# lukecq1231/nats

Measured on NVIDIA H100. Metric: decoder tokens/sec (dim=1000, src=400, |V|=30k) @1/2/4/8 H100 vs Theano CPU, higher is better.
Workload: dtype f32

## Files before the change

### include/nats_b200.h

```cpp
#ifndef NATS_B200_H
#define NATS_B200_H

#include <stdint.h>
#include <stddef.h>

#ifdef __cplusplus
extern "C" {
#endif

#pragma GCC visibility push(default)

#define NATS_NUM_PARAMS 43
#define NATS_GRAD_TAIL 32

typedef struct nats_ctx nats_ctx_t;

typedef struct {
    int32_t n_words;
    int32_t dim_word;
    int32_t dim;
    int32_t dim_att;
} nats_dims_t;

typedef struct {
    char name[32];
    int64_t offset;
    int32_t rows, cols, ld;
    int32_t ndim;
} nats_param_view_t;

const char* nats_last_error(void);
int nats_version(void);

int nats_ctx_create(int device, nats_ctx_t** out);
int nats_ctx_destroy(nats_ctx_t* ctx);

int nats_param_layout(const nats_dims_t* dims, nats_param_view_t* views, int64_t* total_floats);

int64_t nats_train_workspace_bytes(const nats_dims_t* dims, int Tx, int Ty, int B);

int nats_train_fwd(nats_ctx_t* ctx, void* stream, const nats_dims_t* dims, const float* params,
                   const int64_t* x, const float* x_mask, const int64_t* y, const float* y_mask,
                   int Tx, int Ty, int B, void* ws, int64_t ws_bytes, float* cost);

int nats_train_bwd(nats_ctx_t* ctx, void* stream, const nats_dims_t* dims, const float* params,
                   const int64_t* x, const float* x_mask, const int64_t* y, const float* y_mask,
                   int Tx, int Ty, int B, void* ws, int64_t ws_bytes, float scale, float* grads);

int64_t nats_grad_split(const nats_dims_t* dims);
int nats_train_bwd_begin(nats_ctx_t* ctx, void* stream, const nats_dims_t* dims, const float* params,
                         const int64_t* x, const float* x_mask, const int64_t* y, const float* y_mask,
                         int Tx, int Ty, int B, void* ws, int64_t ws_bytes, float scale, float* grads);
int nats_train_bwd_finish(nats_ctx_t* ctx, void* stream, const nats_dims_t* dims, const float* params,
                          const int64_t* x, const float* x_mask, const int64_t* y, const float* y_mask,
                          int Tx, int Ty, int B, void* ws, int64_t ws_bytes, float scale, float* grads);

int nats_encoder_fwd(nats_ctx_t* ctx, void* stream, const nats_dims_t* dims, const float* params,
                     const int64_t* x, const float* x_mask , int Tx, int Ty, int B,
                     void* ws, int64_t ws_bytes);
int nats_decoder_scan_fwd(nats_ctx_t* ctx, void* stream, const nats_dims_t* dims, const float* params,
                          const int64_t* y, const float* x_mask, const float* y_mask, int Tx, int Ty, int B,
                          void* ws, int64_t ws_bytes);
int nats_readout_nll_fwd(nats_ctx_t* ctx, void* stream, const nats_dims_t* dims, const float* params,
                         const int64_t* y, const float* y_mask, int Tx, int Ty, int B,
                         void* ws, int64_t ws_bytes, float* cost);
int nats_readout_nll_bwd(nats_ctx_t* ctx, void* stream, const nats_dims_t* dims, const float* params,
                         const int64_t* y, const float* y_mask, int Tx, int Ty, int B,
                         void* ws, int64_t ws_bytes, float scale, float* grads);
int nats_decoder_scan_bwd(nats_ctx_t* ctx, void* stream, const nats_dims_t* dims, const float* params,
                          const int64_t* y, const float* x_mask, const float* y_mask, int Tx, int Ty, int B,
                          void* ws, int64_t ws_bytes, float* grads);
int nats_encoder_bwd(nats_ctx_t* ctx, void* stream, const nats_dims_t* dims, const float* params,
                     const int64_t* x, const float* x_mask, const int64_t* y, int Tx, int Ty, int B,
                     void* ws, int64_t ws_bytes, float* grads);

const float* nats_train_ws_view(const nats_dims_t* dims, int Tx, int Ty, int B, void* ws, const char* name);

int64_t nats_sampler_workspace_bytes(const nats_dims_t* dims, int Tx, int n);

int nats_sampler_init(nats_ctx_t* ctx, void* stream, const nats_dims_t* dims, const float* params,
                      const int64_t* x, const float* x_mask, int Tx, int n, void* ws, int64_t ws_bytes,
                      float* init_state, float* ctx_out, float* pctx_out);

int nats_sampler_next(nats_ctx_t* ctx, void* stream, const nats_dims_t* dims, const float* params,
                      const int64_t* y, const float* ctx_in, int64_t ctx_tstride, int64_t ctx_bstride,
                      const float* pctx_in, int64_t pctx_tstride, int64_t pctx_bstride,
                      const float* state, const float* acc_ctx, const float* acc_alpha, int Tx, int n,
                      uint64_t rng_seed, uint64_t rng_step, void* ws, int64_t ws_bytes,
                      float* probs, int64_t* sample, float* state_out, float* alphaT, float* ctxs,
                      float* acc_ctx_out, float* acc_alpha_out);

int nats_grad_clip(nats_ctx_t* ctx, void* stream, int64_t n, const float* params, float* grads,
                   float decay_c, float clip_c, float* stats );

int nats_adadelta_grad_shared(nats_ctx_t* ctx, void* stream, int64_t n, const float* zg, float* rg2, float rho);
int nats_adadelta_update(nats_ctx_t* ctx, void* stream, int64_t n, float* params, const float* zg,
                         float* ru2, const float* rg2, float rho, float eps);
int nats_adam_update(nats_ctx_t* ctx, void* stream, int64_t n, float* params, const float* g,
                     float* m, float* v, int64_t step);
int nats_rmsprop_grad_shared(nats_ctx_t* ctx, void* stream, int64_t n, const float* zg, float* rg, float* rg2);
int nats_rmsprop_update(nats_ctx_t* ctx, void* stream, int64_t n, float* params, const float* zg,
                        float* ud, const float* rg, const float* rg2);

int nats_beam_distraction_scores(nats_ctx_t* ctx, void* stream,
                                 const float* hist_alpha, const float* hist_ctx, const float* hist_state,
                                 int len_cap, int hist_len, int live_k, int Tx, int C, int D,
                                 const float* cur_alpha, const float* cur_ctx, const float* cur_state,
                                 float kl_factor, float ctx_factor, float state_factor,
                                 float* scratch, float* out);

int nats_beam_topk(nats_ctx_t* ctx, void* stream, const float* probs , int n, int n_words, int k,
                   int mask_unk, float* out_p , int32_t* out_idx );

int nats_beam_reorder_append(nats_ctx_t* ctx, void* stream, const float* src, float* dst, const float* cur,
                             const int32_t* parent, int n_new, int len_cap, int hist_len, int dim);

int nats_beam_select(nats_ctx_t* ctx, void* stream, const float* top_p, const int32_t* top_i, const float* pen,
                     int k, int maxlen, int step, int32_t* counters, float* scores, int32_t* tokens, int32_t* parents,
                     int64_t* next_w, int32_t* out_tokens, int32_t* out_len, float* out_score, int32_t* fin_parent,
                     int32_t* host_counters);
int nats_beam_advance(nats_ctx_t* ctx, void* stream, const int32_t* parents, const int32_t* fin_parent,
                      const int32_t* counters, int k, int len_cap, int step, int Tx, int C, int D,
                      const float* state_o, float* state_n, const float* acc_ctx_o, float* acc_ctx_n,
                      const float* acc_alpha_o, float* acc_alpha_n,
                      const float* cur_alpha, const float* cur_ctx, const float* cur_state,
                      const float* hist_alpha_src, float* hist_alpha_dst, const float* hist_ctx_src, float* hist_ctx_dst,
                      const float* hist_state_src, float* hist_state_dst, float* out_alpha);

typedef struct nats_beam_step {
    const float* params;
    const int64_t* next_w;
    const float* ctx; const float* pctx;
    int32_t Tx, k, maxlen, use_unk;
    void* ws; int64_t ws_bytes;
    const float* state_in; const float* acc_ctx_in; const float* acc_alpha_in;
    float* probs; float* state_out; float* alphaT; float* ctxs; float* acc_ctx_out; float* acc_alpha_out;
    float kl_factor, ctx_factor, state_factor;
    const float* hist_alpha_in; const float* hist_ctx_in; const float* hist_state_in;
    float* scratch; float* pen;
    float* top_p; int32_t* top_i;
    int32_t* counters; float* scores; int32_t* tokens; int32_t* parents; int32_t* fin_parent;
    int32_t* out_tokens; int32_t* out_len; float* out_score; float* out_alpha; int32_t* host_counters;
    float* state_next; float* acc_ctx_next; float* acc_alpha_next;
    float* hist_alpha_out; float* hist_ctx_out; float* hist_state_out;
} nats_beam_step_t;
int nats_beam_step(nats_ctx_t* ctx, void* stream, const nats_dims_t* dims, const nats_beam_step_t* a, int step);

typedef struct nats_beam_step_many {
    nats_beam_step_t beam;
    int32_t n_src;
    const int32_t* src_len;
} nats_beam_step_many_t;
int nats_beam_step_many(nats_ctx_t* ctx, void* stream, const nats_dims_t* dims, const nats_beam_step_many_t* a, int step);

int nats_debug_gemm(nats_ctx_t* ctx, void* stream, int path, int transA, int transB, int M, int N, int K,
                    const float* A, int lda, const float* B, int ldb, float* C, int ldc, const float* bias,
                    int accumulate, int splitk, int batch, int64_t strideA, int64_t strideB, int64_t strideC);

int nats_profile_enable(nats_ctx_t* ctx, int on);
int nats_profile_num_classes(void);
const char* nats_profile_class_name(int cls);
int nats_profile_read(nats_ctx_t* ctx, int n_classes, double* ms, double* flops, double* bytes, int64_t* launches);

#pragma GCC visibility pop

#ifdef __cplusplus
}
#endif
#endif
```

### nats_b200/_lib.py

```python
import ctypes
import os
from ctypes import (POINTER, Structure, c_char, c_char_p, c_double, c_float, c_int, c_int32, c_int64, c_uint64,
                    c_void_p)

_HERE = os.path.dirname(os.path.abspath(__file__))
LIB_PATH = os.path.join(_HERE, 'libnats_b200.so')
HEADER_PATH = os.path.join(os.path.dirname(_HERE), 'include', 'nats_b200.h')

NUM_PARAMS = 43
GRAD_TAIL = 32


class Dims(Structure):
    _fields_ = [('n_words', c_int32), ('dim_word', c_int32), ('dim', c_int32), ('dim_att', c_int32)]


class ParamView(Structure):
    _fields_ = [('name', c_char * 32), ('offset', c_int64), ('rows', c_int32), ('cols', c_int32),
                ('ld', c_int32), ('ndim', c_int32)]


_P = c_void_p


class BeamStep(Structure):
    _fields_ = ([('params', _P), ('next_w', _P), ('ctx', _P), ('pctx', _P),
                 ('Tx', c_int32), ('k', c_int32), ('maxlen', c_int32), ('use_unk', c_int32),
                 ('ws', _P), ('ws_bytes', c_int64)] +
                [(n, _P) for n in ('state_in', 'acc_ctx_in', 'acc_alpha_in', 'probs', 'state_out', 'alphaT', 'ctxs',
                                   'acc_ctx_out', 'acc_alpha_out')] +
                [('kl_factor', c_float), ('ctx_factor', c_float), ('state_factor', c_float)] +
                [(n, _P) for n in ('hist_alpha_in', 'hist_ctx_in', 'hist_state_in', 'scratch', 'pen', 'top_p', 'top_i',
                                   'counters', 'scores', 'tokens', 'parents', 'fin_parent', 'out_tokens', 'out_len',
                                   'out_score', 'out_alpha', 'host_counters', 'state_next', 'acc_ctx_next',
                                   'acc_alpha_next', 'hist_alpha_out', 'hist_ctx_out', 'hist_state_out')])


class BeamStepMany(Structure):
    _fields_ = [('beam', BeamStep), ('n_src', c_int32), ('src_len', _P)]

SIGNATURES = {
    'nats_last_error': (c_char_p, []),
    'nats_version': (c_int, []),
    'nats_ctx_create': (c_int, [c_int, POINTER(c_void_p)]),
    'nats_ctx_destroy': (c_int, [c_void_p]),
    'nats_param_layout': (c_int, [POINTER(Dims), POINTER(ParamView), POINTER(c_int64)]),
    'nats_train_workspace_bytes': (c_int64, [POINTER(Dims), c_int, c_int, c_int]),
    'nats_train_fwd': (c_int, [c_void_p, _P, POINTER(Dims), _P, _P, _P, _P, _P, c_int, c_int, c_int, _P, c_int64, _P]),
    'nats_train_bwd': (c_int, [c_void_p, _P, POINTER(Dims), _P, _P, _P, _P, _P, c_int, c_int, c_int, _P, c_int64,
                               c_float, _P]),
    'nats_grad_split': (c_int64, [POINTER(Dims)]),
    'nats_train_bwd_begin': (c_int, [c_void_p, _P, POINTER(Dims), _P, _P, _P, _P, _P, c_int, c_int, c_int, _P, c_int64,
                                     c_float, _P]),
    'nats_train_bwd_finish': (c_int, [c_void_p, _P, POINTER(Dims), _P, _P, _P, _P, _P, c_int, c_int, c_int, _P, c_int64,
                                      c_float, _P]),
    'nats_encoder_fwd': (c_int, [c_void_p, _P, POINTER(Dims), _P, _P, _P, c_int, c_int, c_int, _P, c_int64]),
    'nats_decoder_scan_fwd': (c_int, [c_void_p, _P, POINTER(Dims), _P, _P, _P, _P, c_int, c_int, c_int, _P, c_int64]),
    'nats_readout_nll_fwd': (c_int, [c_void_p, _P, POINTER(Dims), _P, _P, _P, c_int, c_int, c_int, _P, c_int64, _P]),
    'nats_readout_nll_bwd': (c_int, [c_void_p, _P, POINTER(Dims), _P, _P, _P, c_int, c_int, c_int, _P, c_int64,
                                     c_float, _P]),
    'nats_decoder_scan_bwd': (c_int, [c_void_p, _P, POINTER(Dims), _P, _P, _P, _P, c_int, c_int, c_int, _P, c_int64,
                                      _P]),
    'nats_encoder_bwd': (c_int, [c_void_p, _P, POINTER(Dims), _P, _P, _P, _P, c_int, c_int, c_int, _P, c_int64, _P]),
    'nats_train_ws_view': (c_void_p, [POINTER(Dims), c_int, c_int, c_int, _P, c_char_p]),
    'nats_sampler_workspace_bytes': (c_int64, [POINTER(Dims), c_int, c_int]),
    'nats_sampler_init': (c_int, [c_void_p, _P, POINTER(Dims), _P, _P, _P, c_int, c_int, _P, c_int64, _P, _P, _P]),
    'nats_sampler_next': (c_int, [c_void_p, _P, POINTER(Dims), _P, _P, _P, c_int64, c_int64, _P, c_int64, c_int64,
                                  _P, _P, _P, c_int, c_int, c_uint64, c_uint64, _P, c_int64,
                                  _P, _P, _P, _P, _P, _P, _P]),
    'nats_grad_clip': (c_int, [c_void_p, _P, c_int64, _P, _P, c_float, c_float, _P]),
    'nats_adadelta_grad_shared': (c_int, [c_void_p, _P, c_int64, _P, _P, c_float]),
    'nats_adadelta_update': (c_int, [c_void_p, _P, c_int64, _P, _P, _P, _P, c_float, c_float]),
    'nats_adam_update': (c_int, [c_void_p, _P, c_int64, _P, _P, _P, _P, c_int64]),
    'nats_rmsprop_grad_shared': (c_int, [c_void_p, _P, c_int64, _P, _P, _P]),
    'nats_rmsprop_update': (c_int, [c_void_p, _P, c_int64, _P, _P, _P, _P, _P]),
    'nats_beam_distraction_scores': (c_int, [c_void_p, _P, _P, _P, _P, c_int, c_int, c_int, c_int, c_int, c_int,
                                             _P, _P, _P, c_float, c_float, c_float, _P, _P]),
    'nats_beam_topk': (c_int, [c_void_p, _P, _P, c_int, c_int, c_int, c_int, _P, _P]),
    'nats_beam_reorder_append': (c_int, [c_void_p, _P, _P, _P, _P, _P, c_int, c_int, c_int, c_int]),
    'nats_beam_select': (c_int, [c_void_p, _P, _P, _P, _P, c_int, c_int, c_int, _P, _P, _P, _P, _P, _P, _P, _P, _P, _P]),
    'nats_beam_advance': (c_int, [c_void_p, _P] + [_P] * 3 + [c_int] * 6 + [_P] * 16),
    'nats_beam_step': (c_int, [c_void_p, _P, POINTER(Dims), POINTER(BeamStep), c_int]),
    'nats_beam_step_many': (c_int, [c_void_p, _P, POINTER(Dims), POINTER(BeamStepMany), c_int]),
    'nats_debug_gemm': (c_int, [c_void_p, _P, c_int, c_int, c_int, c_int, c_int, c_int, _P, c_int, _P, c_int, _P, c_int,
                                _P, c_int, c_int, c_int, c_int64, c_int64, c_int64]),
    'nats_profile_enable': (c_int, [c_void_p, c_int]),
    'nats_profile_num_classes': (c_int, []),
    'nats_profile_class_name': (c_char_p, [c_int]),
    'nats_profile_read': (c_int, [c_void_p, c_int, POINTER(c_double), POINTER(c_double), POINTER(c_double),
                                  POINTER(c_int64)]),
}

_lib = None


class NatsB200Error(RuntimeError):
    pass


def load():
    global _lib
    if _lib is not None:
        return _lib
    if not os.path.exists(LIB_PATH):
        raise NatsB200Error('%s not found: build it with `python nats_b200/csrc/build.py` '
                            '(or __graft_entry__.build()); nats_b200 has no CPU fallback' % LIB_PATH)
    lib = ctypes.CDLL(LIB_PATH)
    for name, (res, args) in SIGNATURES.items():
        fn = getattr(lib, name)
        fn.restype = res
        fn.argtypes = args
    _lib = lib
    return lib


def check(rc, what=''):
    if rc != 0:
        msg = load().nats_last_error()
        raise NatsB200Error('%s failed (rc=%d): %s' % (what or 'libnats_b200 call', rc,
                                                      msg.decode() if msg else '?'))


def param_layout(n_words, dim_word, dim, dim_att):
    lib = load()
    d = Dims(n_words, dim_word, dim, dim_att)
    views = (ParamView * NUM_PARAMS)()
    total = c_int64(0)
    check(lib.nats_param_layout(ctypes.byref(d), views, ctypes.byref(total)), 'nats_param_layout')
    out = [(v.name.decode(), v.offset, v.rows, v.cols, v.ld, v.ndim) for v in views]
    return out, total.value
```

### nats_b200/csrc/api.cu

```cuda
#include <stdarg.h>
#include <stdlib.h>

#include <vector>

#include "model.cuh"

namespace nats {
static thread_local char g_err[1024] = "";
void set_error(const char* fmt, ...) {
    va_list ap;
    va_start(ap, fmt);
    vsnprintf(g_err, sizeof(g_err), fmt, ap);
    va_end(ap);
}
}

namespace nats {
namespace {
struct ProfRec { int cls; double flops, bytes; };
struct ProfState {
    bool on = false;
    std::vector<cudaEvent_t> ev;
    std::vector<ProfRec> recs;
};
ProfState g_prof;
const char* kNames[K_COUNT] = {
    "gemm_big_nn", "gemm_big_nt", "gemm_big_tn", "gemm_big_tt", "gemm_mid_nn", "gemm_mid_nt", "gemm_mid_tn",
    "gemm_mid_tt", "gemm_smallm_nn", "gemm_smallm_nt", "gemm_smallm_tn", "gemm_smallm_tt", "gru_gates_fwd",
    "gru_gates_bwd", "att_scores", "att_context", "att_bwd_ctx", "att_bwd_dalpha", "att_bwd_softmax", "nll_rows",
    "dlogits", "softmax_sample", "colsum", "reduce_splits", "embedding", "elementwise", "optimizer", "beam",
    "memset", "tc_gemm_3xtf32", "tc_gemm_3xtf32_skinny", "enc_tc_fwd", "enc_tc_bwd"};
}
const char* kclass_name(int cls) { return (cls >= 0 && cls < K_COUNT) ? kNames[cls] : "?"; }
bool prof_enabled() { return g_prof.on; }
void prof_begin(cudaStream_t st, int cls, double flops, double bytes) {
    const size_t i = g_prof.recs.size();
    while (g_prof.ev.size() < 2 * (i + 1)) {
        cudaEvent_t e;
        if (cudaEventCreate(&e) != cudaSuccess) { g_prof.on = false; return; }
        g_prof.ev.push_back(e);
    }
    g_prof.recs.push_back(ProfRec{cls, flops, bytes});
    cudaEventRecord(g_prof.ev[2 * i], st);
}
void prof_end(cudaStream_t st) {
    if (g_prof.recs.empty()) return;
    cudaEventRecord(g_prof.ev[2 * (g_prof.recs.size() - 1) + 1], st);
}
}

namespace nats {
static int g_pdl = 1;
int pdl_enabled() { return g_pdl; }
void pdl_set(int on) { g_pdl = on; }
}

using namespace nats;

namespace {

int check_dims(const nats_dims_t* d) {
    NATS_REQUIRE(d != nullptr, "dims");
    NATS_REQUIRE(d->n_words >= 2 && d->dim_word >= 1 && d->dim >= 1 && d->dim_att >= 1, "dims must be positive");
    NATS_REQUIRE(d->dim_att <= 256, "dim_att <= 256");
    return 0;
}

struct ViewDef { const char* name; int64_t off; int rows, cols, ld, ndim; };

}

extern "C" {

const char* nats_last_error(void) { return g_err; }
int nats_version(void) { return 101; }

int nats_ctx_create(int device, nats_ctx_t** out) {
    NATS_REQUIRE(out != nullptr, "out");
    NATS_CUDA_OK(cudaSetDevice(device));
    cudaDeviceProp prop;
    NATS_CUDA_OK(cudaGetDeviceProperties(&prop, device));
    if (prop.major != 9 || prop.minor != 0) {
        set_error("libnats_b200 is built for sm_90a only; device %d is sm_%d%d", device, prop.major, prop.minor);
        return 3;
    }
    nats_ctx* c = new nats_ctx;
    c->device = device;
    c->num_sms = prop.multiProcessorCount;
    c->max_smem_optin = (int)prop.sharedMemPerBlockOptin;
    c->dev_scratch = nullptr;
    NATS_CUDA_OK(cudaMalloc(&c->dev_scratch, kCtxScratchFloats * sizeof(float)));
    int r = attention_setup(c);
    if (r == 0) r = narrow_proj_setup(c);
    if (r == 0) r = tc_gemm_setup();
    if (r == 0) r = tma_gemm_setup();
    if (r == 0) r = enc_tc_setup(c);
    enc_tc_enable(getenv("NATS_ENC_TC") ? atoi(getenv("NATS_ENC_TC")) : 1);
    attention_set_cc_keep(getenv("NATS_CC_KEEP") ? atoi(getenv("NATS_CC_KEEP")) : 0);
    tma_gemm_set_ts(getenv("NATS_TS") ? atoi(getenv("NATS_TS")) : 1);
    if (getenv("NATS_TRACE_GATES")) gates_trace(atoi(getenv("NATS_TRACE_GATES")));
    pdl_set(getenv("NATS_PDL") ? atoi(getenv("NATS_PDL")) : 1);
    gemm_set_tensor_cores(getenv("NATS_TC") ? atoi(getenv("NATS_TC")) : 2);
    if (r != 0) { cudaFree(c->dev_scratch); delete c; return r; }
    *out = c;
    return 0;
}

int nats_ctx_destroy(nats_ctx_t* ctx) {
    if (!ctx) return 0;
    if (ctx->dev_scratch) cudaFree(ctx->dev_scratch);
    delete ctx;
    return 0;
}

int nats_param_layout(const nats_dims_t* dims, nats_param_view_t* views, int64_t* total_floats) {
    NATS_TRY(check_dims(dims));
    const ParamOff o = param_offsets(*dims);
    const int V = dims->n_words, W = dims->dim_word, D = dims->dim, A = dims->dim_att, C = 2 * D, D3 = 3 * D;
    const ViewDef defs[NATS_NUM_PARAMS] = {
        {"Wemb", o.Wemb, V, W, W, 2},
        {"encoder_W", o.enc[0].Wcat, W, 2 * D, D3, 2},
        {"encoder_b", o.enc[0].bcat, 1, 2 * D, D3, 1},
        {"encoder_U", o.enc[0].Ucat, D, 2 * D, D3, 2},
        {"encoder_Wx", o.enc[0].Wcat + 2 * D, W, D, D3, 2},
        {"encoder_bx", o.enc[0].bcat + 2 * D, 1, D, D3, 1},
        {"encoder_Ux", o.enc[0].Ucat + 2 * D, D, D, D3, 2},
        {"encoder_r_W", o.enc[1].Wcat, W, 2 * D, D3, 2},
        {"encoder_r_b", o.enc[1].bcat, 1, 2 * D, D3, 1},
        {"encoder_r_U", o.enc[1].Ucat, D, 2 * D, D3, 2},
        {"encoder_r_Wx", o.enc[1].Wcat + 2 * D, W, D, D3, 2},
        {"encoder_r_bx", o.enc[1].bcat + 2 * D, 1, D, D3, 1},
        {"encoder_r_Ux", o.enc[1].Ucat + 2 * D, D, D, D3, 2},
        {"ff_state_W", o.ff_state_W, C, D, D, 2},
        {"ff_state_b", o.ff_state_b, 1, D, D, 1},
        {"decoder_W", o.dec.Wcat, W, 2 * D, D3, 2},
        {"decoder_U", o.dec.Ucat, D, 2 * D, D3, 2},
        {"decoder_b", o.dec.bcat, 1, 2 * D, D3, 1},
        {"decoder_Wx", o.dec.Wcat + 2 * D, W, D, D3, 2},
        {"decoder_Ux", o.dec.Ucat + 2 * D, D, D, D3, 2},
        {"decoder_bx", o.dec.bcat + 2 * D, 1, D, D3, 1},
        {"decoder_U_1", o.U1cat, D, 2 * D, D3, 2},
        {"decoder_W_1", o.W1cat, C, 2 * D, D3, 2},
        {"decoder_b_1", o.b1cat, 1, 2 * D, D3, 1},
        {"decoder_Wx_1", o.W1cat + 2 * D, C, D, D3, 2},
        {"decoder_Ux_1", o.U1cat + 2 * D, D, D, D3, 2},
        {"decoder_bx_1", o.b1cat + 2 * D, 1, D, D3, 1},
        {"decoder_W_att", o.W_att, D, A, A, 2},
        {"decoder_Wc_att", o.Wc_att, C, A, A, 2},
        {"decoder_b_att", o.b_att, 1, A, A, 1},
        {"decoder_U_att", o.U_att, A, 1, 1, 2},
        {"decoder_c_att", o.c_att, 1, 1, 1, 1},
        {"decoder_W_con", o.W_con, C, 1, 1, 2},
        {"decoder_U_con", o.U_con, C, 1, 1, 2},
        {"decoder_D_wei", o.D_wei, 1, A, A, 2},
        {"ff_logit_lstm_W", o.lstm_W, D, W, W, 2},
        {"ff_logit_lstm_b", o.lstm_b, 1, W, W, 1},
        {"ff_logit_prev_W", o.prev_W, W, W, W, 2},
        {"ff_logit_prev_b", o.prev_b, 1, W, W, 1},
        {"ff_logit_ctx_W", o.ctxr_W, C, W, W, 2},
        {"ff_logit_ctx_b", o.ctxr_b, 1, W, W, 1},
        {"ff_logit_W", o.logit_W, W, V, V, 2},
        {"ff_logit_b", o.logit_b, 1, V, V, 1},
    };
    if (views) {
        for (int i = 0; i < NATS_NUM_PARAMS; ++i) {
            memset(&views[i], 0, sizeof(views[i]));
            strncpy(views[i].name, defs[i].name, sizeof(views[i].name) - 1);
            views[i].offset = defs[i].off;
            views[i].rows = defs[i].rows; views[i].cols = defs[i].cols; views[i].ld = defs[i].ld;
            views[i].ndim = defs[i].ndim;
        }
    }
    if (total_floats) *total_floats = o.total;
    return 0;
}

int nats_debug_gemm(nats_ctx_t* ctx, void* stream, int path, int transA, int transB, int M, int N, int K,
                    const float* A, int lda, const float* B, int ldb, float* C, int ldc, const float* bias,
                    int accumulate, int splitk, int batch, int64_t strideA, int64_t strideB, int64_t strideC) {
    NATS_REQUIRE(ctx && A && B && C, "null argument");
    GemmProblem p = gemm_problem(A, lda, B, ldb, C, ldc, M, N, K);
    p.bias = bias; p.accumulate = accumulate; p.batch = batch < 1 ? 1 : batch;
    p.strideA = strideA; p.strideB = strideB; p.strideC = strideC;
    if (splitk > 1) gemm_set_split(p, splitk, (long long)M * ldc);
    cudaStream_t st = reinterpret_cast<cudaStream_t>(stream);
    if (path == 1) return tc_gemm_launch(st, &p, 1, transA != 0, transB != 0);
    if (path == 2 || path == 3) {
        NATS_REQUIRE(tma_gemm_eligible(&p, 1), "operands not TMA-compatible (alignment)");
        const int keep_ts = tma_gemm_get_ts();
        tma_gemm_set_ts(path == 3 ? 1 : 0);
        const int r = tma_gemm_launch(st, &p, 1, transA != 0, transB != 0);
        tma_gemm_set_ts(keep_ts);
        return r;
    }
    const int keep = gemm_get_tensor_cores();
    gemm_set_tensor_cores(0);
    const int r = gemm_launch(st, &p, 1, transA != 0, transB != 0, GEMM_CFG_AUTO);
    gemm_set_tensor_cores(keep);
    return r;
}

int nats_profile_enable(nats_ctx_t* ctx, int on) {
    (void)ctx;
    g_prof.recs.clear();
    g_prof.on = on != 0;
    return 0;
}
int nats_profile_num_classes(void) { return K_COUNT; }
const char* nats_profile_class_name(int cls) { return kclass_name(cls); }
int nats_profile_read(nats_ctx_t* ctx, int n_classes, double* ms, double* flops, double* bytes, int64_t* launches) {
    (void)ctx;
    NATS_REQUIRE(n_classes >= K_COUNT && ms && flops && bytes && launches, "profile_read buffers");
    NATS_CUDA_OK(cudaDeviceSynchronize());
    for (int i = 0; i < n_classes; ++i) { ms[i] = 0; flops[i] = 0; bytes[i] = 0; launches[i] = 0; }
    for (size_t i = 0; i < g_prof.recs.size(); ++i) {
        float t = 0.f;
        if (cudaEventElapsedTime(&t, g_prof.ev[2 * i], g_prof.ev[2 * i + 1]) != cudaSuccess) continue;
        const ProfRec& r = g_prof.recs[i];
        ms[r.cls] += t; flops[r.cls] += r.flops; bytes[r.cls] += r.bytes; launches[r.cls] += 1;
    }
    g_prof.recs.clear();
    return 0;
}

int64_t nats_train_workspace_bytes(const nats_dims_t* dims, int Tx, int Ty, int B) {
    if (check_dims(dims) != 0 || Tx < 1 || Ty < 1 || B < 1) return -1;
    return carve_train(*dims, Tx, Ty, B, nullptr).bytes;
}

#define NATS_TRAIN_PROLOGUE()                                                                      \
    NATS_REQUIRE(ctx != nullptr, "ctx");                                                           \
    NATS_TRY(check_dims(dims));                                                                    \
    NATS_REQUIRE(Tx >= 1 && Ty >= 1 && B >= 1, "shape");                                           \
    NATS_REQUIRE(ws != nullptr, "workspace");                                                      \
    const TrainWS w = carve_train(*dims, Tx, Ty, B, ws);                                           \
    NATS_REQUIRE(ws_bytes >= w.bytes, "workspace too small (see nats_train_workspace_bytes)");     \
    cudaStream_t st = reinterpret_cast<cudaStream_t>(stream)

int nats_encoder_fwd(nats_ctx_t* ctx, void* stream, const nats_dims_t* dims, const float* params, const int64_t* x,
                     const float* x_mask, int Tx, int Ty, int B, void* ws, int64_t ws_bytes) {
    NATS_TRAIN_PROLOGUE();
    return train_encoder_fwd(ctx, st, *dims, params, x, x_mask, Tx, B, w);
}

int nats_decoder_scan_fwd(nats_ctx_t* ctx, void* stream, const nats_dims_t* dims, const float* params,
                          const int64_t* y, const float* x_mask, const float* y_mask, int Tx, int Ty, int B, void* ws,
                          int64_t ws_bytes) {
    NATS_TRAIN_PROLOGUE();
    return train_decoder_fwd(ctx, st, *dims, params, y, x_mask, y_mask, Tx, Ty, B, w);
}

int nats_readout_nll_fwd(nats_ctx_t* ctx, void* stream, const nats_dims_t* dims, const float* params,
                         const int64_t* y, const float* y_mask, int Tx, int Ty, int B, void* ws, int64_t ws_bytes,
                         float* cost) {
    NATS_TRAIN_PROLOGUE();
    return train_readout_fwd(ctx, st, *dims, params, y, y_mask, Ty, B, w, cost);
}

int nats_readout_nll_bwd(nats_ctx_t* ctx, void* stream, const nats_dims_t* dims, const float* params,
                         const int64_t* y, const float* y_mask, int Tx, int Ty, int B, void* ws, int64_t ws_bytes,
                         float scale, float* grads) {
    NATS_TRAIN_PROLOGUE();
    return train_readout_bwd(ctx, st, *dims, params, y, y_mask, Ty, B, w, scale, grads);
}

int nats_decoder_scan_bwd(nats_ctx_t* ctx, void* stream, const nats_dims_t* dims, const float* params,
                          const int64_t* y, const float* x_mask, const float* y_mask, int Tx, int Ty, int B, void* ws,
                          int64_t ws_bytes, float* grads) {
    NATS_TRAIN_PROLOGUE();
    return train_decoder_bwd(ctx, st, *dims, params, y, x_mask, y_mask, Tx, Ty, B, w, grads);
}

int nats_encoder_bwd(nats_ctx_t* ctx, void* stream, const nats_dims_t* dims, const float* params, const int64_t* x,
                     const float* x_mask, const int64_t* y, int Tx, int Ty, int B, void* ws, int64_t ws_bytes,
                     float* grads) {
    NATS_TRAIN_PROLOGUE();
    return train_encoder_bwd(ctx, st, *dims, params, x, x_mask, y, Tx, Ty, B, w, grads);
}

int nats_train_fwd(nats_ctx_t* ctx, void* stream, const nats_dims_t* dims, const float* params, const int64_t* x,
                   const float* x_mask, const int64_t* y, const float* y_mask, int Tx, int Ty, int B, void* ws,
                   int64_t ws_bytes, float* cost) {
    NATS_TRAIN_PROLOGUE();
    NATS_REQUIRE(x && x_mask && y && y_mask && cost && params, "null argument");
    NATS_TRY(train_encoder_fwd(ctx, st, *dims, params, x, x_mask, Tx, B, w));
    NATS_TRY(train_decoder_fwd(ctx, st, *dims, params, y, x_mask, y_mask, Tx, Ty, B, w));
    NATS_TRY(train_readout_fwd(ctx, st, *dims, params, y, y_mask, Ty, B, w, cost));
    return 0;
}

int64_t nats_grad_split(const nats_dims_t* dims) {
    if (check_dims(dims) != 0) return -1;
    return param_offsets(*dims).ff_state_W;
}

int nats_train_bwd_begin(nats_ctx_t* ctx, void* stream, const nats_dims_t* dims, const float* params, const int64_t* x,
                         const float* x_mask, const int64_t* y, const float* y_mask, int Tx, int Ty, int B, void* ws,
                         int64_t ws_bytes, float scale, float* grads) {
    NATS_TRAIN_PROLOGUE();
    NATS_REQUIRE(x && x_mask && y && y_mask && grads && params, "null argument");
    const ParamOff o = param_offsets(*dims);
    NATS_CUDA_OK(memset_async(st, grads, 0, (size_t)(o.total + NATS_GRAD_TAIL) * sizeof(float)));
    NATS_TRY(cost_reduce(st, w.rowcost, Ty, B, nullptr, scale, grads + o.total));
    NATS_TRY(train_readout_bwd(ctx, st, *dims, params, y, y_mask, Ty, B, w, scale, grads));
    NATS_TRY(train_decoder_bwd(ctx, st, *dims, params, y, x_mask, y_mask, Tx, Ty, B, w, grads));
    return 0;
}

int nats_train_bwd_finish(nats_ctx_t* ctx, void* stream, const nats_dims_t* dims, const float* params, const int64_t* x,
                          const float* x_mask, const int64_t* y, const float* y_mask, int Tx, int Ty, int B, void* ws,
                          int64_t ws_bytes, float scale, float* grads) {
    (void)scale; (void)y_mask;
    NATS_TRAIN_PROLOGUE();
    NATS_REQUIRE(x && x_mask && y && grads && params, "null argument");
    return train_encoder_bwd(ctx, st, *dims, params, x, x_mask, y, Tx, Ty, B, w, grads);
}

int nats_train_bwd(nats_ctx_t* ctx, void* stream, const nats_dims_t* dims, const float* params, const int64_t* x,
                   const float* x_mask, const int64_t* y, const float* y_mask, int Tx, int Ty, int B, void* ws,
                   int64_t ws_bytes, float scale, float* grads) {
    NATS_TRY(nats_train_bwd_begin(ctx, stream, dims, params, x, x_mask, y, y_mask, Tx, Ty, B, ws, ws_bytes, scale, grads));
    return nats_train_bwd_finish(ctx, stream, dims, params, x, x_mask, y, y_mask, Tx, Ty, B, ws, ws_bytes, scale, grads);
}

const float* nats_train_ws_view(const nats_dims_t* dims, int Tx, int Ty, int B, void* ws, const char* name) {
    if (check_dims(dims) != 0 || !ws || !name) return nullptr;
    const TrainWS w = carve_train(*dims, Tx, Ty, B, ws);
    if (!strcmp(name, "ctx")) return w.cc;
    if (!strcmp(name, "init_state")) return w.init_state;
    if (!strcmp(name, "dec_h")) return w.d_h2;
    if (!strcmp(name, "dec_ctx")) return w.d_ctx;
    if (!strcmp(name, "dec_alpha")) return w.d_alpha;
    if (!strcmp(name, "pctx")) return w.pctx;
    if (!strcmp(name, "logits")) return w.logits;
    return nullptr;
}

int64_t nats_sampler_workspace_bytes(const nats_dims_t* dims, int Tx, int n) {
    if (check_dims(dims) != 0 || Tx < 1 || n < 1) return -1;
    return carve_sampler(*dims, Tx, n, nullptr).bytes;
}

int nats_sampler_init(nats_ctx_t* ctx, void* stream, const nats_dims_t* dims, const float* params, const int64_t* x,
                      const float* x_mask, int Tx, int n, void* ws, int64_t ws_bytes, float* init_state, float* ctx_out,
                      float* pctx_out) {
    NATS_REQUIRE(ctx && ws && params && x && init_state && ctx_out, "null argument");
    NATS_TRY(check_dims(dims));
    NATS_REQUIRE(Tx >= 1 && n >= 1, "shape");
    const SamplerWS w = carve_sampler(*dims, Tx, n, ws);
    NATS_REQUIRE(ws_bytes >= w.bytes, "workspace too small (see nats_sampler_workspace_bytes)");
    cudaStream_t st = reinterpret_cast<cudaStream_t>(stream);
    EncBufs e;
    memset(&e, 0, sizeof(e));
    e.emb_x = w.emb_x;
    e.xproj[0] = w.xproj[0]; e.xproj[1] = w.xproj[1];
    e.cc = ctx_out; e.ctxsum = w.ctxsum; e.xlen = w.xlen; e.xinv = w.xinv; e.ctx_mean = w.ctx_mean;
    e.init_state = init_state; e.part_a = w.part_a;
    e.gemm_scratch = w.gemm_scratch; e.gemm_scratch_floats = w.gemm_scratch_floats;
    e.enc_scratch = w.enc_scratch; e.enc_scratch_floats = w.enc_scratch_floats;
    e.enc_counters = w.enc_counters; e.enc_counter_ints = w.enc_counter_ints;
    NATS_TRY(encoder_forward(ctx, st, *dims, params, x, x_mask, Tx, n, e));
    if (pctx_out) {
        const ParamOff o = param_offsets(*dims);
        const int A = dims->dim_att, C = 2 * dims->dim;
        GemmProblem p = gemm_problem(ctx_out, C, params + o.Wc_att, A, pctx_out, A, Tx * n, A, C);
        p.bias = params + o.b_att;
        NATS_TRY(gemm_auto(ctx, st, p, false, false, w.gemm_scratch, w.gemm_scratch_floats));
    }
    return 0;
}

}

namespace {

int sampler_next(nats_ctx_t* ctx, void* stream, const nats_dims_t* dims, const float* params, const int64_t* y,
                 const float* ctx_in, int64_t ctx_tstride, int64_t ctx_bstride, const float* pctx_in,
                 int64_t pctx_tstride, int64_t pctx_bstride, int rows_per_src, const int32_t* src_len, const float* state,
                 const float* acc_ctx, const float* acc_alpha, int Tx, int n, uint64_t rng_seed, uint64_t rng_step, void* ws,
                 int64_t ws_bytes, float* probs, int64_t* sample, float* state_out, float* alphaT, float* ctxs,
                 float* acc_ctx_out, float* acc_alpha_out) {
    NATS_REQUIRE(ctx && ws && params && y && ctx_in && state && acc_ctx && acc_alpha, "null argument");
    NATS_REQUIRE(probs && state_out && alphaT && ctxs && acc_ctx_out && acc_alpha_out, "null output");
    NATS_TRY(check_dims(dims));
    NATS_REQUIRE(Tx >= 1 && n >= 1, "shape");
    const SamplerWS w = carve_sampler(*dims, Tx, n, ws);
    NATS_REQUIRE(ws_bytes >= w.bytes, "workspace too small (see nats_sampler_workspace_bytes)");
    cudaStream_t st = reinterpret_cast<cudaStream_t>(stream);
    const ParamOff o = param_offsets(*dims);
    const int W = dims->dim_word, D = dims->dim, A = dims->dim_att, V = dims->n_words, C = 2 * D, D3 = 3 * D;

    NATS_TRY(gather_rows(st, params + o.Wemb, y, n, W, V, 0, w.emb_y));
    {
        GemmProblem p = gemm_problem(w.emb_y, W, params + o.dec.Wcat, D3, w.xproj_y, D3, n, D3, W);
        p.bias = params + o.dec.bcat;
        NATS_TRY(gemm_auto(ctx, st, p, false, false, w.gemm_scratch, w.gemm_scratch_floats));
    }
    const float* pctx = pctx_in;
    long long pts = pctx_tstride, pbs = pctx_bstride;
    if (!pctx) {
        GemmProblem p;
        if (ctx_bstride == 0) {
            p = gemm_problem(ctx_in, (int)ctx_tstride, params + o.Wc_att, A, w.pctx, A, Tx, A, C);
            pts = A; pbs = 0;
        } else {
            NATS_REQUIRE(ctx_bstride == C && ctx_tstride == (int64_t)n * C, "pctx recompute needs a dense [Tx,n,C] context");
            p = gemm_problem(ctx_in, C, params + o.Wc_att, A, w.pctx, A, Tx * n, A, C);
            pts = (long long)n * A; pbs = A;
        }
        p.bias = params + o.b_att;
        NATS_TRY(gemm_auto(ctx, st, p, false, false, w.gemm_scratch, w.gemm_scratch_floats));
        pctx = w.pctx;
    }
    DecStep s;
    memset(&s, 0, sizeof(s));
    s.n = n; s.Tx = Tx;
    s.h_prev = state; s.xproj = w.xproj_y;
    s.ymask = nullptr; s.xmask = nullptr;
    s.rows_per_src = rows_per_src; s.src_len = src_len;
    s.pctx = pctx; s.pctx_ts = pts; s.pctx_bs = pbs;
    s.cc = ctx_in; s.cc_ts = ctx_tstride; s.cc_bs = ctx_bstride;
    s.acc_alpha_in = acc_alpha; s.acc_ctx_in = acc_ctx;
    s.h1 = w.h1; s.ps_save = w.ps; s.escore = w.escore;
    s.alpha_out = alphaT; s.acc_alpha_out = acc_alpha_out; s.craw_out = w.craw; s.ctx_out = ctxs;
    s.acc_ctx_out = acc_ctx_out; s.h2 = state_out;
    s.part_a = w.part_a; s.part_b = w.part_b; s.part_c = w.part_c; s.part_d = w.part_d;
    NATS_TRY(decoder_step_forward(ctx, st, *dims, params, s));

    NarrowProj np;
    memset(&np, 0, sizeof(np));
    np.x[0] = state_out; np.ldx[0] = D; np.W[0] = params + o.lstm_W; np.ldw[0] = W; np.bias[0] = params + o.lstm_b; np.K[0] = D;
    np.x[1] = w.emb_y;   np.ldx[1] = W; np.W[1] = params + o.prev_W; np.ldw[1] = W; np.bias[1] = params + o.prev_b; np.K[1] = W;
    np.x[2] = ctxs;      np.ldx[2] = C; np.W[2] = params + o.ctxr_W; np.ldw[2] = W; np.bias[2] = params + o.ctxr_b; np.K[2] = C;
    np.n = n; np.N = W; np.out = w.L; np.ldo = W; np.act_tanh = 1;
    GemmProblem p;
    if (narrow_proj_eligible(np)) {
        NATS_TRY(narrow_proj(st, np));
    } else {
        p = gemm_problem(state_out, D, params + o.lstm_W, W, w.L, W, n, W, D);
        p.bias = params + o.lstm_b;
        NATS_TRY(gemm_auto(ctx, st, p, false, false, w.gemm_scratch, w.gemm_scratch_floats));
        p = gemm_problem(w.emb_y, W, params + o.prev_W, W, w.L, W, n, W, W);
        p.bias = params + o.prev_b; p.accumulate = 1;
        NATS_TRY(gemm_auto(ctx, st, p, false, false, w.gemm_scratch, w.gemm_scratch_floats));
        p = gemm_problem(ctxs, C, params + o.ctxr_W, W, w.L, W, n, W, C);
        p.bias = params + o.ctxr_b; p.accumulate = 1;
        NATS_TRY(gemm_auto(ctx, st, p, false, false, w.gemm_scratch, w.gemm_scratch_floats));
        NATS_TRY(tanh_inplace(st, w.L, (long long)n * W));
    }
    p = gemm_problem(w.L, W, params + o.logit_W, V, w.logits, V, n, V, W);
    p.bias = params + o.logit_b;
    NATS_TRY(gemm_auto(ctx, st, p, false, false, w.gemm_scratch, w.gemm_scratch_floats));
    NATS_TRY(softmax_sample_rows(st, w.logits, n, V, probs, sample, rng_seed, rng_step));
    return 0;
}

}

extern "C" {

int nats_sampler_next(nats_ctx_t* ctx, void* stream, const nats_dims_t* dims, const float* params, const int64_t* y,
                      const float* ctx_in, int64_t ctx_tstride, int64_t ctx_bstride, const float* pctx_in,
                      int64_t pctx_tstride, int64_t pctx_bstride, const float* state, const float* acc_ctx,
                      const float* acc_alpha, int Tx, int n, uint64_t rng_seed, uint64_t rng_step, void* ws,
                      int64_t ws_bytes, float* probs, int64_t* sample, float* state_out, float* alphaT, float* ctxs,
                      float* acc_ctx_out, float* acc_alpha_out) {
    return sampler_next(ctx, stream, dims, params, y, ctx_in, ctx_tstride, ctx_bstride, pctx_in, pctx_tstride, pctx_bstride,
                        ctx_bstride == 0 ? n : 1, nullptr, state, acc_ctx, acc_alpha, Tx, n, rng_seed, rng_step, ws, ws_bytes,
                        probs, sample, state_out, alphaT, ctxs, acc_ctx_out, acc_alpha_out);
}

int nats_grad_clip(nats_ctx_t* ctx, void* stream, int64_t n, const float* params, float* grads, float decay_c,
                   float clip_c, float* stats) {
    NATS_REQUIRE(ctx && grads && stats, "null argument");
    NATS_REQUIRE(!(decay_c > 0.f) || params, "params needed for decay");
    return grad_clip(ctx, reinterpret_cast<cudaStream_t>(stream), n, params, grads, decay_c, clip_c, stats);
}
int nats_adadelta_grad_shared(nats_ctx_t* ctx, void* stream, int64_t n, const float* zg, float* rg2, float rho) {
    (void)ctx;
    return adadelta_grad_shared(reinterpret_cast<cudaStream_t>(stream), n, zg, rg2, rho);
}
int nats_adadelta_update(nats_ctx_t* ctx, void* stream, int64_t n, float* params, const float* zg, float* ru2,
                         const float* rg2, float rho, float eps) {
    (void)ctx;
    return adadelta_update(reinterpret_cast<cudaStream_t>(stream), n, params, zg, ru2, rg2, rho, eps);
}
int nats_adam_update(nats_ctx_t* ctx, void* stream, int64_t n, float* params, const float* g, float* m, float* v,
                     int64_t step) {
    (void)ctx;
    return adam_update(reinterpret_cast<cudaStream_t>(stream), n, params, g, m, v, step);
}
int nats_rmsprop_grad_shared(nats_ctx_t* ctx, void* stream, int64_t n, const float* zg, float* rg, float* rg2) {
    (void)ctx;
    return rmsprop_grad_shared(reinterpret_cast<cudaStream_t>(stream), n, zg, rg, rg2);
}
int nats_rmsprop_update(nats_ctx_t* ctx, void* stream, int64_t n, float* params, const float* zg, float* ud,
                        const float* rg, const float* rg2) {
    (void)ctx;
    return rmsprop_update(reinterpret_cast<cudaStream_t>(stream), n, params, zg, ud, rg, rg2);
}

int nats_beam_distraction_scores(nats_ctx_t* ctx, void* stream, const float* hist_alpha, const float* hist_ctx,
                                 const float* hist_state, int len_cap, int hist_len, int live_k, int Tx, int C, int D,
                                 const float* cur_alpha, const float* cur_ctx, const float* cur_state, float kl_factor,
                                 float ctx_factor, float state_factor, float* scratch, float* out) {
    (void)ctx;
    return beam_distraction_scores(reinterpret_cast<cudaStream_t>(stream), hist_alpha, hist_ctx, hist_state, len_cap,
                                   hist_len, live_k, Tx, C, D, cur_alpha, cur_ctx, cur_state, kl_factor, ctx_factor,
                                   state_factor, nullptr, 0, scratch, out);
}
int nats_beam_topk(nats_ctx_t* ctx, void* stream, const float* probs, int n, int n_words, int k, int mask_unk,
                   float* out_p, int32_t* out_idx) {
    (void)ctx;
    return beam_topk(reinterpret_cast<cudaStream_t>(stream), probs, n, n_words, k, mask_unk, out_p, out_idx);
}

int nats_beam_reorder_append(nats_ctx_t* ctx, void* stream, const float* src, float* dst, const float* cur,
                             const int32_t* parent, int n_new, int len_cap, int hist_len, int dim) {
    (void)ctx;
    return beam_reorder_append(reinterpret_cast<cudaStream_t>(stream), src, dst, cur, parent, n_new, len_cap, hist_len,
                               dim);
}

int nats_beam_select(nats_ctx_t* ctx, void* stream, const float* top_p, const int32_t* top_i, const float* pen, int k,
                     int maxlen, int step, int32_t* counters, float* scores, int32_t* tokens, int32_t* parents,
                     int64_t* next_w, int32_t* out_tokens, int32_t* out_len, float* out_score, int32_t* fin_parent,
                     int32_t* host_counters) {
    (void)ctx;
    NATS_REQUIRE(top_p && top_i && counters && scores && tokens && parents && next_w && out_tokens && out_len && out_score &&
                     fin_parent, "null argument");
    return beam_select(reinterpret_cast<cudaStream_t>(stream), top_p, top_i, pen, 1, k, maxlen, step, counters, scores, tokens,
                       parents, reinterpret_cast<long long*>(next_w), out_tokens, out_len, out_score, fin_parent, host_counters);
}

int nats_beam_advance(nats_ctx_t* ctx, void* stream, const int32_t* parents, const int32_t* fin_parent,
                      const int32_t* counters, int k, int len_cap, int step, int Tx, int C, int D, const float* state_o,
                      float* state_n, const float* acc_ctx_o, float* acc_ctx_n, const float* acc_alpha_o, float* acc_alpha_n,
                      const float* cur_alpha, const float* cur_ctx, const float* cur_state, const float* hist_alpha_src,
                      float* hist_alpha_dst, const float* hist_ctx_src, float* hist_ctx_dst, const float* hist_state_src,
                      float* hist_state_dst, float* out_alpha) {
    (void)ctx;
    NATS_REQUIRE(parents && fin_parent && counters && state_o && state_n && acc_ctx_o && acc_ctx_n && acc_alpha_o &&
                     acc_alpha_n && cur_alpha && hist_alpha_src && hist_alpha_dst && out_alpha, "null argument");
    NATS_REQUIRE(hist_ctx_src == nullptr || (hist_ctx_dst && hist_state_src && hist_state_dst && cur_ctx && cur_state),
                 "context / state histories come together");
    return beam_advance(reinterpret_cast<cudaStream_t>(stream), parents, fin_parent, counters, 1, k, len_cap, step, Tx, C, D,
                        state_o, state_n, acc_ctx_o, acc_ctx_n, acc_alpha_o, acc_alpha_n, cur_alpha, cur_ctx, cur_state,
                        hist_alpha_src, hist_alpha_dst, hist_ctx_src, hist_ctx_dst, hist_state_src, hist_state_dst, out_alpha);
}

}

namespace {

int beam_step_group(nats_ctx_t* ctx, cudaStream_t st, const nats_dims_t* dims, const nats_beam_step_t* a, int n_src,
                    const int32_t* src_len, int step) {
    NATS_REQUIRE(ctx && dims && a, "null argument");
    NATS_REQUIRE(a->k >= 1 && a->k <= 32 && a->maxlen >= 1 && step >= 0 && step < a->maxlen, "beam step shape (1 <= k <= 32)");
    NATS_REQUIRE(n_src >= 1 && (long long)n_src * a->k <= 65535, "beam group size");
    NATS_TRY(check_dims(dims));
    const int D = dims->dim, C = 2 * D, A = dims->dim_att, V = dims->n_words, k = a->k, Tx = a->Tx, n = n_src * k;
    void* stream = reinterpret_cast<void*>(st);
    const int64_t cbs = n_src == 1 ? 0 : C, pbs = n_src == 1 ? 0 : A;
    NATS_TRY(sampler_next(ctx, stream, dims, a->params, a->next_w, a->ctx, (int64_t)n_src * C, cbs, a->pctx, (int64_t)n_src * A,
                          pbs, k, src_len, a->state_in, a->acc_ctx_in, a->acc_alpha_in, Tx, n, 0, 0, a->ws, a->ws_bytes,
                          a->probs, nullptr, a->state_out, a->alphaT, a->ctxs, a->acc_ctx_out, a->acc_alpha_out));
    const bool distract = a->kl_factor > 0.f || a->ctx_factor > 0.f || a->state_factor > 0.f;
    const bool use_pen = distract && step > 0;
    if (use_pen) {
        NATS_REQUIRE(a->hist_ctx_in && a->hist_state_in && a->scratch && a->pen, "distraction buffers");
        NATS_TRY(beam_distraction_scores(st, a->hist_alpha_in, a->hist_ctx_in, a->hist_state_in, a->maxlen, step, n, Tx, C, D,
                                         a->alphaT, a->ctxs, a->state_out, a->kl_factor, a->ctx_factor, a->state_factor,
                                         a->counters, k, a->scratch, a->pen));
    }
    NATS_REQUIRE(a->probs && a->top_p && a->top_i && a->counters && a->scores && a->tokens && a->parents && a->next_w &&
                     a->out_tokens && a->out_len && a->out_score && a->fin_parent, "null argument");
    NATS_REQUIRE(a->state_next && a->acc_ctx_next && a->acc_alpha_next && a->hist_alpha_in && a->hist_alpha_out && a->out_alpha,
                 "null argument");
    NATS_REQUIRE(!distract || (a->hist_ctx_out && a->hist_state_out), "distraction histories");
    NATS_TRY(beam_topk(st, a->probs, n, V, k, a->use_unk ? 0 : 1, a->top_p, a->top_i));
    NATS_TRY(beam_select(st, a->top_p, a->top_i, use_pen ? a->pen : nullptr, n_src, k, a->maxlen, step, a->counters, a->scores,
                         a->tokens, a->parents, reinterpret_cast<long long*>(const_cast<int64_t*>(a->next_w)), a->out_tokens,
                         a->out_len, a->out_score, a->fin_parent, a->host_counters));
    NATS_TRY(beam_advance(st, a->parents, a->fin_parent, a->counters, n_src, k, a->maxlen, step, Tx, C, D, a->state_out,
                          a->state_next, a->acc_ctx_out, a->acc_ctx_next, a->acc_alpha_out, a->acc_alpha_next, a->alphaT, a->ctxs,
                          a->state_out, a->hist_alpha_in, a->hist_alpha_out, distract ? a->hist_ctx_in : nullptr,
                          a->hist_ctx_out, a->hist_state_in, a->hist_state_out, a->out_alpha));
    return 0;
}

}

extern "C" {

int nats_beam_step(nats_ctx_t* ctx, void* stream, const nats_dims_t* dims, const nats_beam_step_t* a, int step) {
    return beam_step_group(ctx, reinterpret_cast<cudaStream_t>(stream), dims, a, 1, nullptr, step);
}

int nats_beam_step_many(nats_ctx_t* ctx, void* stream, const nats_dims_t* dims, const nats_beam_step_many_t* a, int step) {
    NATS_REQUIRE(a != nullptr, "null argument");
    NATS_REQUIRE(a->n_src >= 1, "n_src >= 1");
    NATS_REQUIRE(a->src_len != nullptr, "src_len");
    return beam_step_group(ctx, reinterpret_cast<cudaStream_t>(stream), dims, &a->beam, a->n_src, a->src_len, step);
}


}
```

### nats_b200/csrc/gemm.cuh

```cuda
#pragma once
#include "common.cuh"

namespace nats {


struct GemmProblem {
    const float* A;
    const float* B;
    float* C;
    const float* bias;
    int M, N, K;
    int lda, ldb, ldc;
    int batch;
    long long strideA, strideB, strideC;
    int splitk;
    int kchunk;
    long long strideP;
    int accumulate;
};

constexpr int kGemmMaxGroup = 4;
constexpr int kGemmMaxSplit = 32;

struct GemmGroup {
    GemmProblem p[kGemmMaxGroup];
    int zstart[kGemmMaxGroup + 1];
    int count;
};

enum GemmCfg { GEMM_CFG_AUTO = 0, GEMM_CFG_BIG = 1, GEMM_CFG_MID = 2, GEMM_CFG_SMALLM = 3 };

inline GemmProblem gemm_problem(const float* A, int lda, const float* B, int ldb, float* C, int ldc,
                                int M, int N, int K) {
    GemmProblem p;
    memset(&p, 0, sizeof(p));
    p.A = A; p.B = B; p.C = C; p.bias = nullptr;
    p.M = M; p.N = N; p.K = K; p.lda = lda; p.ldb = ldb; p.ldc = ldc;
    p.batch = 1; p.splitk = 1; p.kchunk = ((K + 15) / 16) * 16; if (p.kchunk == 0) p.kchunk = 16;
    p.accumulate = 0;
    return p;
}
inline void gemm_set_split(GemmProblem& p, int splits, long long strideP) {
    if (splits < 1) splits = 1;
    int chunk = (p.K + splits - 1) / splits;
    chunk = ((chunk + 15) / 16) * 16;
    if (chunk == 0) chunk = 16;
    p.kchunk = chunk;
    p.splitk = splits;
    p.strideP = strideP;
}

int tc_gemm_launch(cudaStream_t st, const GemmProblem* probs, int count, bool transA, bool transB);
int tc_gemm_setup();
int tma_gemm_launch(cudaStream_t st, const GemmProblem* probs, int count, bool transA, bool transB);
bool tma_gemm_eligible(const GemmProblem* probs, int count);
int tma_gemm_setup();
void gemm_set_tensor_cores(int on);
int gemm_get_tensor_cores();

int gemm_launch(cudaStream_t st, const GemmProblem* probs, int count, bool transA, bool transB, int cfg);

int gemm_step_cfg(int M);
int gemm_pick_split(const nats_ctx* ctx, int M, int N, int K, int groups = 1);

int gemm_auto(const nats_ctx* ctx, cudaStream_t st, GemmProblem p, bool transA, bool transB,
              float* scratch, long long scratch_floats);

int reduce_splits(cudaStream_t st, const float* part, int nsplit, long long strideP, int M, int N, int ldp,
                  float* out, int ldo, const float* bias, int accumulate);

}
```

### nats_b200/csrc/model_bwd.cu

```cuda
#include "model.cuh"

namespace nats {

namespace {
inline int ga(const nats_ctx* ctx, cudaStream_t st, const TrainWS& w, GemmProblem p, bool ta, bool tb) {
    return gemm_auto(ctx, st, p, ta, tb, w.gemm_scratch, w.gemm_scratch_floats);
}
}

int train_readout_bwd(const nats_ctx* ctx, cudaStream_t st, const nats_dims_t& d, const float* params,
                      const int64_t* y, const float* y_mask, int Ty, int B, const TrainWS& w, float scale,
                      float* G) {
    const ParamOff o = param_offsets(d);
    const int W = d.dim_word, D = d.dim, V = d.n_words, C = 2 * D;
    const int YB = Ty * B;
    NATS_TRY(dlogits_inplace(st, w.logits, YB, V, y, y_mask, w.lse, scale));
    NATS_TRY(ga(ctx, st, w, gemm_problem(w.L, W, w.logits, V, G + o.logit_W, V, W, V, YB), true, false));
    NATS_TRY(colsum(st, w.logits, YB, V, V, G + o.logit_b, 0, w.red_scratch));
    NATS_TRY(ga(ctx, st, w, gemm_problem(w.logits, V, params + o.logit_W, V, w.dpre, W, YB, W, V), false, true));
    NATS_TRY(dtanh(st, w.dpre, w.L, w.dpre, (long long)YB * W));
    NATS_TRY(ga(ctx, st, w, gemm_problem(w.d_h2, D, w.dpre, W, G + o.lstm_W, W, D, W, YB), true, false));
    NATS_TRY(ga(ctx, st, w, gemm_problem(w.embs, W, w.dpre, W, G + o.prev_W, W, W, W, YB), true, false));
    NATS_TRY(ga(ctx, st, w, gemm_problem(w.d_ctx, C, w.dpre, W, G + o.ctxr_W, W, C, W, YB), true, false));
    NATS_TRY(colsum3(st, w.dpre, YB, W, W, G + o.lstm_b, G + o.prev_b, G + o.ctxr_b, 0, w.red_scratch));
    NATS_TRY(ga(ctx, st, w, gemm_problem(w.dpre, W, params + o.lstm_W, W, w.dh2_ro, D, YB, D, W), false, true));
    NATS_TRY(ga(ctx, st, w, gemm_problem(w.dpre, W, params + o.ctxr_W, W, w.dctx_ro, C, YB, C, W), false, true));
    NATS_TRY(ga(ctx, st, w, gemm_problem(w.dpre, W, params + o.prev_W, W, w.dembs, W, YB, W, W), false, true));
    return 0;
}

int train_decoder_bwd(const nats_ctx* ctx, cudaStream_t st, const nats_dims_t& d, const float* params,
                      const int64_t* y, const float* x_mask, const float* y_mask, int Tx, int Ty, int B,
                      const TrainWS& w, float* G) {
    const ParamOff o = param_offsets(d);
    const int W = d.dim_word, D = d.dim, A = d.dim_att, V = d.n_words, C = 2 * D, D3 = 3 * D;
    const long long XB = (long long)Tx * B, YB = (long long)Ty * B;
    const int cfg = gemm_step_cfg(B);
    const int SA = gemm_pick_split(ctx, B, D, D3);
    const int SB = gemm_pick_split(ctx, B, C, D3);
    const int S4 = gemm_pick_split(ctx, B, D, D3);
    const long long spD = (long long)B * D, spC = (long long)B * C;

    NATS_CUDA_OK(memset_async(st, w.dpctx, 0, (size_t)XB * A * sizeof(float)));
    NATS_CUDA_OK(memset_async(st, w.dacc_alpha, 0, (size_t)B * Tx * sizeof(float)));
    NATS_CUDA_OK(memset_async(st, w.dacc_ctx, 0, (size_t)2 * B * C * sizeof(float)));
    NATS_CUDA_OK(memset_async(st, w.gatt_part, 0, (size_t)B * (2 * A + 1) * sizeof(float)));

    for (int t = Ty - 1; t >= 0; --t) {
        const long long rD = (long long)t * B * D, rC = (long long)t * B * C, rT = (long long)t * B * Tx;
        const long long r3 = (long long)t * B * D3, rA = (long long)t * B * A;
        const float* ym = y_mask + (long long)t * B;
        const int pp = t & 1;
        {
            GateBwd g;
            memset(&g, 0, sizeof(g));
            g.dh_a = w.dh2_ro + rD; g.ld_a = D;
            if (t < Ty - 1) {
                g.dh_b = w.dh_elem; g.ld_b = D;
                g.part = w.part_c; g.nsplit = S4; g.part_stride = spD; g.part_ld = D;
            }
            g.r = w.d_r2 + rD; g.u = w.d_u2 + rD; g.c = w.d_c2 + rD; g.p = w.d_p2 + rD;
            g.h_prev = w.d_h1 + rD; g.ld_hprev = D;
            g.mask = ym;
            g.dG = w.dG1 + r3; g.dGx = w.dG1x + r3; g.dh_elem = w.dh1_elem;
            NATS_TRY(gru_gates_bwd(st, &g, 1, B, D));
        }
        {
            GemmProblem q[2];
            q[0] = gemm_problem(w.dG1 + r3, D3, params + o.U1cat, D3, w.part_b, D, B, D, D3);
            gemm_set_split(q[0], SA, spD);
            q[1] = gemm_problem(w.dG1x + r3, D3, params + o.W1cat, D3, w.part_a, C, B, C, D3);
            gemm_set_split(q[1], SB, spC);
            NATS_TRY(gemm_launch(st, q, 2, false, true, cfg));
        }
        {
            AttBwd a;
            memset(&a, 0, sizeof(a));
            a.pctx = w.pctx; a.cc = w.cc;
            a.dctx_a = w.dctx_ro + rC;
            a.dctx_part = w.part_a; a.dctx_nsplit = SB; a.dctx_stride = spC;
            a.dacc_ctx_in = w.dacc_ctx + (long long)pp * B * C;
            a.dacc_ctx_out = w.dacc_ctx + (long long)(pp ^ 1) * B * C;
            a.dacc_alpha = w.dacc_alpha;
            a.ymask = ym;
            a.ctx = w.d_ctx + rC; a.craw = w.d_craw + rC; a.acc_ctx = w.d_accctx + rC;
            a.alpha = w.d_alpha + rT; a.acc_alpha = w.d_accalpha + rT;
            a.ps = w.d_ps + rA;
            a.D_wei = params + o.D_wei; a.U_att = params + o.U_att; a.U_con = params + o.U_con; a.W_con = params + o.W_con;
            a.dq = w.dq + rC; a.dcraw = w.dcraw + rC;
            a.dalpha = w.dalpha;
            a.dps = w.dps + rA;
            a.dpctx = w.dpctx;
            a.gatt_part = w.gatt_part;
            a.dot_part = w.att_dot_part; a.soft_part = w.att_soft_part;
            a.Tx = Tx; a.B = B; a.A = A; a.C = C;
            NATS_TRY(attention_bwd(ctx, st, a));
        }
        {
            GemmProblem q = gemm_problem(w.dps + rA, A, params + o.W_att, A, w.part_d, D, B, D, A);
            NATS_TRY(gemm_launch(st, &q, 1, false, true, cfg));
        }
        {
            GateBwd g;
            memset(&g, 0, sizeof(g));
            g.dh_a = w.dh1_elem; g.ld_a = D;
            g.part = w.part_b; g.nsplit = SA; g.part_stride = spD; g.part_ld = D;
            g.part2 = w.part_d; g.nsplit2 = 1; g.part2_stride = spD; g.part2_ld = D;
            g.r = w.d_r1 + rD; g.u = w.d_u1 + rD; g.c = w.d_c1 + rD; g.p = w.d_p1 + rD;
            g.h_prev = t > 0 ? w.d_h2 + rD - spD : w.init_state; g.ld_hprev = D;
            g.mask = ym;
            g.dG = w.dG2 + r3; g.dGx = w.dG2x + r3; g.dh_elem = w.dh_elem;
            NATS_TRY(gru_gates_bwd(st, &g, 1, B, D));
        }
        {
            GemmProblem q = gemm_problem(w.dG2 + r3, D3, params + o.dec.Ucat, D3, w.part_c, D, B, D, D3);
            gemm_set_split(q, S4, spD);
            NATS_TRY(gemm_launch(st, &q, 1, false, true, cfg));
        }
    }
    NATS_TRY(sum_parts_dtanh(st, w.dh_elem, w.part_c, S4, spD, w.init_state, w.dinit, B, D));

    {
        NATS_TRY(ga(ctx, st, w, gemm_problem(w.init_state, D, w.dG2, D3, G + o.dec.Ucat, D3, D, D3, B), true, false));
        if (Ty > 1) {
            GemmProblem p = gemm_problem(w.d_h2, D, w.dG2 + (long long)B * D3, D3, G + o.dec.Ucat, D3, D, D3, (Ty - 1) * B);
            p.accumulate = 1;
            NATS_TRY(ga(ctx, st, w, p, true, false));
        }
    }
    NATS_TRY(ga(ctx, st, w, gemm_problem(w.embs, W, w.dG2x, D3, G + o.dec.Wcat, D3, W, D3, (int)YB), true, false));
    NATS_TRY(colsum(st, w.dG2x, YB, D3, D3, G + o.dec.bcat, 0, w.red_scratch));
    NATS_TRY(ga(ctx, st, w, gemm_problem(w.d_h1, D, w.dG1, D3, G + o.U1cat, D3, D, D3, (int)YB), true, false));
    NATS_TRY(ga(ctx, st, w, gemm_problem(w.d_ctx, C, w.dG1x, D3, G + o.W1cat, D3, C, D3, (int)YB), true, false));
    NATS_TRY(colsum(st, w.dG1, YB, D3, D3, G + o.b1cat, 0, w.red_scratch));
    NATS_TRY(ga(ctx, st, w, gemm_problem(w.d_h1, D, w.dps, A, G + o.W_att, A, D, A, (int)YB), true, false));
    NATS_TRY(ga(ctx, st, w, gemm_problem(w.cc, C, w.dpctx, A, G + o.Wc_att, A, C, A, (int)XB), true, false));
    NATS_TRY(colsum(st, w.dpctx, XB, A, A, G + o.b_att, 0, w.red_scratch));
    NATS_TRY(colsum_prod(st, w.dq, w.d_craw, YB, C, C, G + o.U_con, 0, w.red_scratch));
    NATS_TRY(colsum_prod(st, w.dq, w.d_accctx, YB, C, C, G + o.W_con, 0, w.red_scratch));
    NATS_TRY(colsum(st, w.gatt_part, B, A, 2 * A + 1, G + o.U_att, 0, w.red_scratch));
    NATS_TRY(colsum(st, w.gatt_part + A, B, A, 2 * A + 1, G + o.D_wei, 0, w.red_scratch));
    NATS_TRY(colsum(st, w.gatt_part + 2 * A, B, 1, 2 * A + 1, G + o.c_att, 0, w.red_scratch));

    NATS_TRY(ga(ctx, st, w, gemm_problem(w.dpctx, A, params + o.Wc_att, A, w.dcc, C, (int)XB, C, A), false, true));
    {
        GemmProblem p = gemm_problem(w.d_alpha, B * Tx, w.dcraw, B * C, w.dcc, B * C, Tx, C, Ty);
        p.batch = B; p.strideA = Tx; p.strideB = C; p.strideC = C; p.accumulate = 1;
        NATS_TRY(gemm_launch(st, &p, 1, true, false, GEMM_CFG_AUTO));
    }
    {
        GemmProblem p = gemm_problem(w.dG2x, D3, params + o.dec.Wcat, D3, w.dembs, W, (int)YB, W, D3);
        p.accumulate = 1;
        NATS_TRY(ga(ctx, st, w, p, false, true));
        NATS_TRY(scatter_add_rows(st, G + o.Wemb, y, (int)YB, W, V, B, w.dembs));
    }
    NATS_TRY(ga(ctx, st, w, gemm_problem(w.ctx_mean, C, w.dinit, D, G + o.ff_state_W, D, C, D, B), true, false));
    NATS_TRY(colsum(st, w.dinit, B, D, D, G + o.ff_state_b, 0, w.red_scratch));
    NATS_TRY(ga(ctx, st, w, gemm_problem(w.dinit, D, params + o.ff_state_W, D, w.dmean, C, B, C, D), false, true));
    return 0;
}

int train_encoder_bwd(const nats_ctx* ctx, cudaStream_t st, const nats_dims_t& d, const float* params,
                      const int64_t* x, const float* x_mask, const int64_t* y, int Tx, int Ty, int B,
                      const TrainWS& w, float* G) {
    (void)y; (void)Ty;
    const ParamOff o = param_offsets(d);
    const int W = d.dim_word, D = d.dim, V = d.n_words, C = 2 * D, D3 = 3 * D;
    const long long XB = (long long)Tx * B;
    const int cfg = gemm_step_cfg(B);
    const int S = gemm_pick_split(ctx, B, D, D3, 2);
    const long long strideP = 2LL * B * D;
    const bool persistent = enc_tc_eligible(ctx, B, D, 1);
    if (persistent) {
        EncTcBwdArgs pa;
        memset(&pa, 0, sizeof(pa));
        for (int dir = 0; dir < 2; ++dir) {
            pa.Ucat[dir] = params + o.enc[dir].Ucat;
            pa.r[dir] = w.enc_r[dir]; pa.u[dir] = w.enc_u[dir]; pa.c[dir] = w.enc_c[dir]; pa.p[dir] = w.enc_p[dir];
            pa.dG[dir] = w.dGe[dir]; pa.dGx[dir] = w.dGex[dir];
        }
        pa.dcc = w.dcc; pa.mean_grad = w.dmean; pa.coef = w.xinv; pa.mask = x_mask; pa.cc = w.cc;
        pa.bar = w.enc_counters; pa.bar_ints = w.enc_counter_ints;
        pa.scratch = w.enc_scratch; pa.scratch_floats = w.enc_scratch_floats;
        pa.Tx = Tx; pa.n = B; pa.D = D;
        NATS_TRY(enc_tc_bwd(ctx, st, pa));
    }
    for (int s = Tx - 1; s >= 0 && !persistent; --s) {
        const int pf = s, pb = Tx - 1 - s;
        GateBwd g[2];
        memset(g, 0, sizeof(g));
        for (int dir = 0; dir < 2; ++dir) {
            const int pos = dir == 0 ? pf : pb;
            const int prev = dir == 0 ? pf - 1 : pb + 1;
            const long long so = (long long)pos * B * D;
            g[dir].dh_a = w.dcc + (long long)pos * B * C + dir * D; g[dir].ld_a = C;
            if (s < Tx - 1) {
                g[dir].dh_b = w.dh_elem + (long long)dir * B * D; g[dir].ld_b = D;
                g[dir].part = w.part_a + (long long)dir * B * D; g[dir].nsplit = S;
                g[dir].part_stride = strideP; g[dir].part_ld = D;
            }
            g[dir].mean_grad = w.dmean + dir * D; g[dir].ld_mean = C; g[dir].coef = w.xinv;
            g[dir].r = w.enc_r[dir] + so; g[dir].u = w.enc_u[dir] + so; g[dir].c = w.enc_c[dir] + so;
            g[dir].p = w.enc_p[dir] + so;
            g[dir].h_prev = s > 0 ? w.cc + (long long)prev * B * C + dir * D : nullptr; g[dir].ld_hprev = C;
            g[dir].mask = x_mask + (long long)pos * B;
            g[dir].dG = w.dGe[dir] + (long long)pos * B * D3;
            g[dir].dGx = w.dGex[dir] + (long long)pos * B * D3;
            g[dir].dh_elem = w.dh_elem + (long long)dir * B * D;
        }
        NATS_TRY(gru_gates_bwd(st, g, 2, B, D));
        if (s > 0) {
            GemmProblem q[2];
            for (int dir = 0; dir < 2; ++dir) {
                const int pos = dir == 0 ? pf : pb;
                q[dir] = gemm_problem(w.dGe[dir] + (long long)pos * B * D3, D3, params + o.enc[dir].Ucat, D3,
                                      w.part_a + (long long)dir * B * D, D, B, D, D3);
                gemm_set_split(q[dir], S, strideP);
            }
            NATS_TRY(gemm_launch(st, q, 2, false, true, cfg));
        }
    }
    if (Tx > 1) {
        const int K = (Tx - 1) * B;
        NATS_TRY(ga(ctx, st, w, gemm_problem(w.cc, C, w.dGe[0] + (long long)B * D3, D3, G + o.enc[0].Ucat, D3, D, D3, K),
                    true, false));
        NATS_TRY(ga(ctx, st, w, gemm_problem(w.cc + (long long)B * C + D, C, w.dGe[1], D3, G + o.enc[1].Ucat, D3, D, D3, K),
                    true, false));
    }
    for (int dir = 0; dir < 2; ++dir) {
        NATS_TRY(ga(ctx, st, w, gemm_problem(w.emb_x, W, w.dGex[dir], D3, G + o.enc[dir].Wcat, D3, W, D3, (int)XB),
                    true, false));
        NATS_TRY(colsum(st, w.dGex[dir], XB, D3, D3, G + o.enc[dir].bcat, 0, w.red_scratch));
        GemmProblem p = gemm_problem(w.dGex[dir], D3, params + o.enc[dir].Wcat, D3, w.demb_x, W, (int)XB, W, D3);
        p.accumulate = dir;
        NATS_TRY(ga(ctx, st, w, p, false, true));
    }
    NATS_TRY(scatter_add_rows(st, G + o.Wemb, x, (int)XB, W, V, 0, w.demb_x));
    return 0;
}

}
```

### nats_b200/csrc/model_fwd.cu

```cuda
#include "model.cuh"

namespace nats {

int encoder_forward(const nats_ctx* ctx, cudaStream_t st, const nats_dims_t& d, const float* params,
                    const int64_t* x, const float* x_mask, int Tx, int n, const EncBufs& e) {
    const ParamOff o = param_offsets(d);
    const int W = d.dim_word, D = d.dim, V = d.n_words, C = 2 * D, D3 = 3 * D;
    const long long XB = (long long)Tx * n;
    NATS_TRY(gather_rows(st, params + o.Wemb, x, (int)XB, W, V, 0, e.emb_x));
    {
        GemmProblem pr[2];
        for (int dir = 0; dir < 2; ++dir) {
            pr[dir] = gemm_problem(e.emb_x, W, params + o.enc[dir].Wcat, D3, e.xproj[dir], D3, (int)XB, D3, W);
            pr[dir].bias = params + o.enc[dir].bcat;
        }
        NATS_TRY(gemm_launch(st, pr, 2, false, false, GEMM_CFG_AUTO));
    }
    NATS_CUDA_OK(memset_async(st, e.ctxsum, 0, (size_t)n * C * sizeof(float)));
    const int S = gemm_pick_split(ctx, n, D3, D, 2);
    const int cfg = gemm_step_cfg(n);
    const long long strideP = 2LL * n * D3;
    if (enc_tc_eligible(ctx, n, D, 0) && e.enc_scratch != nullptr) {
        EncTcFwdArgs pa;
        memset(&pa, 0, sizeof(pa));
        for (int dir = 0; dir < 2; ++dir) {
            pa.Ucat[dir] = params + o.enc[dir].Ucat; pa.xproj[dir] = e.xproj[dir];
            pa.r[dir] = e.r[dir]; pa.u[dir] = e.u[dir]; pa.c[dir] = e.c[dir]; pa.p[dir] = e.p[dir];
        }
        pa.mask = x_mask; pa.cc = e.cc; pa.ctxsum = e.ctxsum;
        pa.bar = e.enc_counters; pa.bar_ints = e.enc_counter_ints;
        pa.scratch = e.enc_scratch; pa.scratch_floats = e.enc_scratch_floats;
        pa.Tx = Tx; pa.n = n; pa.D = D;
        NATS_TRY(enc_tc_fwd(ctx, st, pa));
    } else {
        for (int s = 0; s < Tx; ++s) {
            const int pf = s, pb = Tx - 1 - s;
            if (s > 0) {
                GemmProblem q[2];
                q[0] = gemm_problem(e.cc + (long long)(pf - 1) * n * C, C, params + o.enc[0].Ucat, D3, e.part_a, D3, n, D3, D);
                q[1] = gemm_problem(e.cc + (long long)(pb + 1) * n * C + D, C, params + o.enc[1].Ucat, D3,
                                    e.part_a + (long long)n * D3, D3, n, D3, D);
                gemm_set_split(q[0], S, strideP);
                gemm_set_split(q[1], S, strideP);
                NATS_TRY(gemm_launch(st, q, 2, false, false, cfg));
            }
            GateFwd g[2];
            memset(g, 0, sizeof(g));
            for (int dir = 0; dir < 2; ++dir) {
                const int pos = dir == 0 ? pf : pb;
                const int prev = dir == 0 ? pf - 1 : pb + 1;
                g[dir].part = e.part_a + (long long)dir * n * D3;
                g[dir].nsplit = s > 0 ? S : 0;
                g[dir].part_stride = strideP;
                g[dir].xproj = e.xproj[dir] + (long long)pos * n * D3;
                g[dir].h_prev = s > 0 ? e.cc + (long long)prev * n * C + dir * D : nullptr;
                g[dir].ld_hprev = C;
                g[dir].mask = x_mask ? x_mask + (long long)pos * n : nullptr;
                g[dir].h_out = e.cc + (long long)pos * n * C + dir * D;
                g[dir].ld_hout = C;
                if (e.r[dir]) {
                    const long long so = (long long)pos * n * D;
                    g[dir].r = e.r[dir] + so; g[dir].u = e.u[dir] + so; g[dir].c = e.c[dir] + so; g[dir].p = e.p[dir] + so;
                }
                g[dir].ctxsum = e.ctxsum + dir * D;
                g[dir].ld_ctxsum = C;
            }
            NATS_TRY(gru_gates_fwd(st, g, 2, n, D, 0));
        }
    }
    NATS_TRY(mask_lengths(st, x_mask, Tx, n, e.xlen, e.xinv));
    NATS_TRY(scale_rows(st, e.ctxsum, e.xinv, n, C, e.ctx_mean));
    GemmProblem pi = gemm_problem(e.ctx_mean, C, params + o.ff_state_W, D, e.init_state, D, n, D, C);
    pi.bias = params + o.ff_state_b;
    NATS_TRY(gemm_auto(ctx, st, pi, false, false, e.gemm_scratch, e.gemm_scratch_floats));
    NATS_TRY(tanh_inplace(st, e.init_state, (long long)n * D));
    return 0;
}

int decoder_step_forward(const nats_ctx* ctx, cudaStream_t st, const nats_dims_t& d, const float* params,
                         const DecStep& s) {
    const ParamOff o = param_offsets(d);
    const int D = d.dim, A = d.dim_att, C = 2 * D, D3 = 3 * D, n = s.n;
    const int cfg = gemm_step_cfg(n);
    const int S1 = gemm_pick_split(ctx, n, D3, D);
    const int S2 = gemm_pick_split(ctx, n, D3, C);
    const long long sp3 = (long long)n * D3;
    {
        GemmProblem q = gemm_problem(s.h_prev, D, params + o.dec.Ucat, D3, s.part_b, D3, n, D3, D);
        gemm_set_split(q, S1, sp3);
        NATS_TRY(gemm_launch(st, &q, 1, false, false, cfg));
        GateFwd g;
        memset(&g, 0, sizeof(g));
        g.part = s.part_b; g.nsplit = S1; g.part_stride = sp3;
        g.xproj = s.xproj;
        g.h_prev = s.h_prev; g.ld_hprev = D;
        g.mask = s.ymask;
        g.h_out = s.h1; g.ld_hout = D;
        g.r = s.r1; g.u = s.u1; g.c = s.c1; g.p = s.p1;
        NATS_TRY(gru_gates_fwd(st, &g, 1, n, D, 0));
    }
    {
        GemmProblem q[2];
        q[0] = gemm_problem(s.h1, D, params + o.U1cat, D3, s.part_c, D3, n, D3, D);
        gemm_set_split(q[0], S1, sp3);
        q[1] = gemm_problem(s.h1, D, params + o.W_att, A, s.part_d, A, n, A, D);
        gemm_set_split(q[1], S1, (long long)n * A);
        NATS_TRY(gemm_launch(st, q, 2, false, false, cfg));
    }
    {
        AttFwd a;
        memset(&a, 0, sizeof(a));
        a.pctx = s.pctx; a.pctx_tstride = s.pctx_ts; a.pctx_bstride = s.pctx_bs;
        a.cc = s.cc; a.cc_tstride = s.cc_ts; a.cc_bstride = s.cc_bs;
        a.ps_part = s.part_d; a.ps_nsplit = S1; a.ps_stride = (long long)n * A;
        a.ps_save = s.ps_save;
        a.acc_alpha_in = s.acc_alpha_in; a.acc_ctx_in = s.acc_ctx_in;
        a.xmask = s.xmask; a.ymask = s.ymask;
        a.rows_per_src = s.rows_per_src; a.src_len = s.src_len;
        a.D_wei = params + o.D_wei; a.U_att = params + o.U_att; a.c_att = params + o.c_att;
        a.U_con = params + o.U_con; a.W_con = params + o.W_con;
        a.escore = s.escore;
        a.alpha_out = s.alpha_out; a.acc_alpha_out = s.acc_alpha_out;
        a.craw_out = s.craw_out; a.ctx_out = s.ctx_out; a.acc_ctx_out = s.acc_ctx_out;
        a.Tx = s.Tx; a.n = n; a.A = A; a.C = C;
        NATS_TRY(attention_fwd(ctx, st, a));
    }
    {
        GemmProblem q = gemm_problem(s.ctx_out, C, params + o.W1cat, D3, s.part_a, D3, n, D3, C);
        gemm_set_split(q, S2, sp3);
        NATS_TRY(gemm_launch(st, &q, 1, false, false, cfg));
        GateFwd g;
        memset(&g, 0, sizeof(g));
        g.part = s.part_c; g.nsplit = S1; g.part_stride = sp3;
        g.part2 = s.part_a; g.nsplit2 = S2; g.part2_stride = sp3;
        g.bias = params + o.b1cat;
        g.h_prev = s.h1; g.ld_hprev = D;
        g.mask = s.ymask;
        g.h_out = s.h2; g.ld_hout = D;
        g.r = s.r2; g.u = s.u2; g.c = s.c2; g.p = s.p2;
        NATS_TRY(gru_gates_fwd(st, &g, 1, n, D, 1));
    }
    return 0;
}

int train_encoder_fwd(const nats_ctx* ctx, cudaStream_t st, const nats_dims_t& d, const float* params,
                      const int64_t* x, const float* x_mask, int Tx, int B, const TrainWS& w) {
    EncBufs e;
    memset(&e, 0, sizeof(e));
    e.emb_x = w.emb_x;
    for (int i = 0; i < 2; ++i) {
        e.xproj[i] = w.xproj[i];
        e.r[i] = w.enc_r[i]; e.u[i] = w.enc_u[i]; e.c[i] = w.enc_c[i]; e.p[i] = w.enc_p[i];
    }
    e.cc = w.cc; e.ctxsum = w.ctxsum; e.xlen = w.xlen; e.xinv = w.xinv; e.ctx_mean = w.ctx_mean;
    e.init_state = w.init_state; e.part_a = w.part_a;
    e.gemm_scratch = w.gemm_scratch; e.gemm_scratch_floats = w.gemm_scratch_floats;
    e.enc_scratch = w.enc_scratch; e.enc_scratch_floats = w.enc_scratch_floats;
    e.enc_counters = w.enc_counters; e.enc_counter_ints = w.enc_counter_ints;
    return encoder_forward(ctx, st, d, params, x, x_mask, Tx, B, e);
}

int train_decoder_fwd(const nats_ctx* ctx, cudaStream_t st, const nats_dims_t& d, const float* params,
                      const int64_t* y, const float* x_mask, const float* y_mask, int Tx, int Ty, int B,
                      const TrainWS& w) {
    const ParamOff o = param_offsets(d);
    const int W = d.dim_word, D = d.dim, A = d.dim_att, V = d.n_words, C = 2 * D, D3 = 3 * D;
    const long long XB = (long long)Tx * B, YB = (long long)Ty * B;
    NATS_TRY(gather_rows(st, params + o.Wemb, y, (int)YB, W, V, B, w.embs));
    {
        GemmProblem p = gemm_problem(w.embs, W, params + o.dec.Wcat, D3, w.xproj_y, D3, (int)YB, D3, W);
        p.bias = params + o.dec.bcat;
        NATS_TRY(gemm_auto(ctx, st, p, false, false, w.gemm_scratch, w.gemm_scratch_floats));
    }
    {
        GemmProblem p = gemm_problem(w.cc, C, params + o.Wc_att, A, w.pctx, A, (int)XB, A, C);
        p.bias = params + o.b_att;
        NATS_TRY(gemm_auto(ctx, st, p, false, false, w.gemm_scratch, w.gemm_scratch_floats));
    }
    NATS_CUDA_OK(memset_async(st, w.d_accalpha, 0, (size_t)B * Tx * sizeof(float)));
    NATS_CUDA_OK(memset_async(st, w.d_accctx, 0, (size_t)B * C * sizeof(float)));
    for (int t = 0; t < Ty; ++t) {
        const long long rD = (long long)t * B * D, rC = (long long)t * B * C, rT = (long long)t * B * Tx;
        DecStep s;
        memset(&s, 0, sizeof(s));
        s.n = B; s.Tx = Tx;
        s.h_prev = t == 0 ? w.init_state : w.d_h2 + rD - (long long)B * D;
        s.xproj = w.xproj_y + (long long)t * B * D3;
        s.ymask = y_mask + (long long)t * B;
        s.xmask = x_mask;
        s.pctx = w.pctx; s.pctx_ts = (long long)B * A; s.pctx_bs = A;
        s.cc = w.cc; s.cc_ts = (long long)B * C; s.cc_bs = C;
        s.acc_alpha_in = w.d_accalpha + rT; s.acc_alpha_out = w.d_accalpha + rT + (long long)B * Tx;
        s.acc_ctx_in = w.d_accctx + rC; s.acc_ctx_out = w.d_accctx + rC + (long long)B * C;
        s.h1 = w.d_h1 + rD; s.r1 = w.d_r1 + rD; s.u1 = w.d_u1 + rD; s.c1 = w.d_c1 + rD; s.p1 = w.d_p1 + rD;
        s.ps_save = w.d_ps + (long long)t * B * A;
        s.escore = w.escore;
        s.alpha_out = w.d_alpha + rT;
        s.craw_out = w.d_craw + rC; s.ctx_out = w.d_ctx + rC;
        s.r2 = w.d_r2 + rD; s.u2 = w.d_u2 + rD; s.c2 = w.d_c2 + rD; s.p2 = w.d_p2 + rD; s.h2 = w.d_h2 + rD;
        s.part_a = w.part_a; s.part_b = w.part_b; s.part_c = w.part_c; s.part_d = w.part_d;
        NATS_TRY(decoder_step_forward(ctx, st, d, params, s));
    }
    return 0;
}

int train_readout_fwd(const nats_ctx* ctx, cudaStream_t st, const nats_dims_t& d, const float* params,
                      const int64_t* y, const float* y_mask, int Ty, int B, const TrainWS& w, float* cost) {
    const ParamOff o = param_offsets(d);
    const int W = d.dim_word, D = d.dim, V = d.n_words, C = 2 * D;
    const int YB = Ty * B;
    GemmProblem p = gemm_problem(w.d_h2, D, params + o.lstm_W, W, w.L, W, YB, W, D);
    p.bias = params + o.lstm_b;
    NATS_TRY(gemm_auto(ctx, st, p, false, false, w.gemm_scratch, w.gemm_scratch_floats));
    p = gemm_problem(w.embs, W, params + o.prev_W, W, w.L, W, YB, W, W);
    p.bias = params + o.prev_b; p.accumulate = 1;
    NATS_TRY(gemm_auto(ctx, st, p, false, false, w.gemm_scratch, w.gemm_scratch_floats));
    p = gemm_problem(w.d_ctx, C, params + o.ctxr_W, W, w.L, W, YB, W, C);
    p.bias = params + o.ctxr_b; p.accumulate = 1;
    NATS_TRY(gemm_auto(ctx, st, p, false, false, w.gemm_scratch, w.gemm_scratch_floats));
    NATS_TRY(tanh_inplace(st, w.L, (long long)YB * W));
    p = gemm_problem(w.L, W, params + o.logit_W, V, w.logits, V, YB, V, W);
    p.bias = params + o.logit_b;
    NATS_TRY(gemm_auto(ctx, st, p, false, false, w.gemm_scratch, w.gemm_scratch_floats));
    NATS_TRY(nll_rows(st, w.logits, YB, V, y, y_mask, w.lse, w.rowcost));
    NATS_TRY(cost_reduce(st, w.rowcost, Ty, B, cost, 1.f, nullptr));
    return 0;
}

}
```

### nats_b200/csrc/ops.cuh

```cuda
#pragma once
#include "common.cuh"

namespace nats {

int gather_rows(cudaStream_t st, const float* Wemb, const int64_t* ids, int n_rows, int W, int V, int shift,
                float* out);
int scatter_add_rows(cudaStream_t st, float* dWemb, const int64_t* ids, int n_rows, int W, int V, int shift,
                     const float* src);

struct GateFwd {
    const float* part;
    int nsplit;
    long long part_stride;
    const float* xproj;
    const float* part2;
    int nsplit2;
    long long part2_stride;
    const float* bias;
    const float* h_prev;
    int ld_hprev;
    const float* mask;
    float* h_out;
    int ld_hout;
    float* r; float* u; float* c; float* p;
    float* ctxsum;
    int ld_ctxsum;
};
int gru_gates_fwd(cudaStream_t st, const GateFwd* groups, int ngroups, int B, int D, int mode);

struct GateBwd {
    const float* dh_a; int ld_a;
    const float* dh_b; int ld_b;
    const float* part;  int nsplit;  long long part_stride;  int part_ld;
    const float* part2; int nsplit2; long long part2_stride; int part2_ld;
    const float* mean_grad; int ld_mean;
    const float* coef;
    const float* r; const float* u; const float* c; const float* p;
    const float* h_prev; int ld_hprev;
    const float* mask;
    float* dG;
    float* dGx;
    float* dh_elem;
};
int gru_gates_bwd(cudaStream_t st, const GateBwd* groups, int ngroups, int B, int D);

struct EncTcFwdArgs {
    const float* Ucat[2]; const float* xproj[2]; const float* mask; float* cc;
    float* r[2]; float* u[2]; float* c[2]; float* p[2];
    float* ctxsum;
    unsigned* bar; long long bar_ints;
    float* scratch; long long scratch_floats;
    unsigned long long* dbg;
    int Tx, n, D;
};
struct EncTcBwdArgs {
    const float* Ucat[2]; const float* dcc; const float* mean_grad; const float* coef; const float* mask; const float* cc;
    const float* r[2]; const float* u[2]; const float* c[2]; const float* p[2];
    float* dG[2]; float* dGx[2];
    unsigned* bar; long long bar_ints; float* scratch; long long scratch_floats;
    unsigned long long* dbg;
    int Tx, n, D;
};
bool enc_tc_eligible(const nats_ctx* ctx, int n, int D, int pass);
void enc_tc_enable(int on);
int enc_tc_setup(const nats_ctx* ctx);
long long enc_tc_scratch_floats(int n, int D);
long long enc_tc_counter_ints();
int enc_tc_fwd(const nats_ctx* ctx, cudaStream_t st, const EncTcFwdArgs& a);
int enc_tc_bwd(const nats_ctx* ctx, cudaStream_t st, const EncTcBwdArgs& a);
void tma_gemm_set_ts(int on);
int tma_gemm_get_ts();
void gates_trace(int on);
void attention_set_cc_keep(int mode);

int tanh_inplace(cudaStream_t st, float* x, long long n);
struct NarrowProj {
    const float* x[3]; long long ldx[3];
    const float* W[3]; long long ldw[3];
    const float* bias[3];
    int K[3];
    int n, N;
    float* out; long long ldo;
    int act_tanh;
};
int narrow_proj_setup(const nats_ctx* ctx);
bool narrow_proj_eligible(const NarrowProj& a);
int narrow_proj(cudaStream_t st, const NarrowProj& a);
int dtanh(cudaStream_t st, const float* g, const float* y, float* dst, long long n);
int sum_parts_dtanh(cudaStream_t st, const float* a, const float* part, int nsplit, long long part_stride,
                    const float* y, float* dst, int B, int D);
int mask_lengths(cudaStream_t st, const float* mask, int Tx, int B, float* xlen, float* inv);
int scale_rows(cudaStream_t st, const float* src, const float* inv, int B, int C, float* out);
int colsum(cudaStream_t st, const float* X, long long K, int N, int ld, float* out, int accumulate, float* scratch);
int colsum3(cudaStream_t st, const float* X, long long K, int N, int ld, float* out, float* out2, float* out3, int accumulate,
            float* scratch);
int colsum_prod(cudaStream_t st, const float* X, const float* Y, long long K, int N, int ld, float* out,
                int accumulate, float* scratch);
int cost_reduce(cudaStream_t st, const float* rowcost, int Ty, int B, float* cost, float scale, float* total);

struct AttFwd {
    const float* pctx; long long pctx_tstride, pctx_bstride;
    const float* cc;   long long cc_tstride, cc_bstride;
    int cc_keep;
    const float* ps_part; int ps_nsplit; long long ps_stride;
    float* ps_save;
    const float* acc_alpha_in;
    const float* acc_ctx_in;
    const float* xmask;
    int rows_per_src;
    const int32_t* src_len;
    const float* ymask;
    const float* D_wei; const float* U_att; const float* c_att; const float* U_con; const float* W_con;
    float* escore;
    float* alpha_out;
    float* acc_alpha_out;
    float* craw_out;
    float* ctx_out;
    float* acc_ctx_out;
    int Tx, n, A, C;
};
int attention_fwd(const nats_ctx* ctx, cudaStream_t st, const AttFwd& a);
int attention_setup(const nats_ctx* ctx);

struct AttBwd {
    const float* pctx; const float* cc;
    int cc_keep;
    const float* dctx_a;
    const float* dctx_part; int dctx_nsplit; long long dctx_stride;
    const float* dacc_ctx_in; float* dacc_ctx_out;
    float* dacc_alpha;
    const float* ymask;
    const float* ctx; const float* craw; const float* acc_ctx;
    const float* alpha; const float* acc_alpha;
    const float* ps;
    const float* D_wei; const float* U_att; const float* U_con; const float* W_con;
    float* dq; float* dcraw;
    float* dalpha;
    float* dps;
    float* dpctx;
    float* gatt_part;
    float* dot_part;
    float* soft_part;
    int Tx, B, A, C;
};
int attention_bwd(const nats_ctx* ctx, cudaStream_t st, const AttBwd& a);

int nll_rows(cudaStream_t st, const float* logits, int rows, int V, const int64_t* y, const float* ymask,
             float* lse, float* rowcost);
int dlogits_inplace(cudaStream_t st, float* logits, int rows, int V, const int64_t* y, const float* ymask,
                    const float* lse, float scale);
int softmax_sample_rows(cudaStream_t st, const float* logits, int rows, int V, float* probs, int64_t* sample,
                        uint64_t seed, uint64_t step);

int grad_clip(const nats_ctx* ctx, cudaStream_t st, long long n, const float* params, float* grads, float decay_c,
              float clip_c, float* stats);
int adadelta_grad_shared(cudaStream_t st, long long n, const float* zg, float* rg2, float rho);
int adadelta_update(cudaStream_t st, long long n, float* p, const float* zg, float* ru2, const float* rg2,
                    float rho, float eps);
int adam_update(cudaStream_t st, long long n, float* p, const float* g, float* m, float* v, long long step);
int rmsprop_grad_shared(cudaStream_t st, long long n, const float* zg, float* rg, float* rg2);
int rmsprop_update(cudaStream_t st, long long n, float* p, const float* zg, float* ud, const float* rg,
                   const float* rg2);

int beam_distraction_scores(cudaStream_t st, const float* hist_alpha, const float* hist_ctx, const float* hist_state,
                            int len_cap, int hist_len, int live_k, int Tx, int C, int D, const float* cur_alpha,
                            const float* cur_ctx, const float* cur_state, float kl, float cf, float sf,
                            const int32_t* counters, int k, float* scratch, float* out);
int beam_topk(cudaStream_t st, const float* probs, int n, int V, int K, int mask_unk, float* out_p, int32_t* out_idx);
int beam_reorder_append(cudaStream_t st, const float* src, float* dst, const float* cur, const int32_t* parent,
                        int n_new, int len_cap, int hist_len, int dim);
int beam_select(cudaStream_t st, const float* top_p, const int32_t* top_i, const float* pen, int n_src, int k, int maxlen,
                int step, int32_t* counters, float* scores, int32_t* tokens, int32_t* parents, long long* next_w,
                int32_t* out_tokens, int32_t* out_len, float* out_score, int32_t* fin_parent, int32_t* host_counters);
int beam_advance(cudaStream_t st, const int32_t* parents, const int32_t* fin_parent, const int32_t* counters, int n_src,
                 int k, int len_cap, int step, int Tx, int C, int D, const float* state_o, float* state_n, const float* acc_ctx_o,
                 float* acc_ctx_n, const float* acc_alpha_o, float* acc_alpha_n, const float* cur_alpha, const float* cur_ctx,
                 const float* cur_state, const float* hist_alpha_src, float* hist_alpha_dst, const float* hist_ctx_src,
                 float* hist_ctx_dst, const float* hist_state_src, float* hist_state_dst, float* out_alpha);

}
```

### nats_b200/csrc/tma_gemm.cu

```cuda
#include <cuda.h>

#include <unordered_map>

#include "gemm.cuh"
#include "ops.cuh"
#include "tc_common.cuh"

namespace nats {

namespace {

typedef CUresult (*EncodeTiledFn)(CUtensorMap*, CUtensorMapDataType, cuuint32_t, void*, const cuuint64_t*,
                                  const cuuint64_t*, const cuuint32_t*, const cuuint32_t*, CUtensorMapInterleave,
                                  CUtensorMapSwizzle, CUtensorMapL2promotion, CUtensorMapFloatOOBfill);
EncodeTiledFn g_encode = nullptr;

struct MapKey {
    const void* ptr; long long inner, outer, ld, batch, bstride; int box_outer; int mn;
    bool operator==(const MapKey& o) const {
        return ptr == o.ptr && inner == o.inner && outer == o.outer && ld == o.ld && batch == o.batch &&
               bstride == o.bstride && box_outer == o.box_outer && mn == o.mn;
    }
};
struct MapKeyHash {
    size_t operator()(const MapKey& k) const {
        size_t h = std::hash<const void*>()(k.ptr);
        auto mix = [&](long long v) { h ^= std::hash<long long>()(v) + 0x9e3779b97f4a7c15ull + (h << 6) + (h >> 2); };
        mix(k.inner); mix(k.outer); mix(k.ld); mix(k.batch); mix(k.bstride); mix(k.box_outer); mix(k.mn);
        return h;
    }
};
std::unordered_map<MapKey, CUtensorMap, MapKeyHash> g_maps;


constexpr int kThreads = 256;
constexpr int kBlockK = 32;
constexpr int kNR = 3;
constexpr int kMaxGroup = 2;

struct TmaProblem {
    float* C;
    const float* bias;
    int Ma, Nb, K;
    long long c_rs, c_cs;
    int batch;
    long long sC;
    int splitk, kchunk;
    long long strideP;
    int accumulate;
    int bias_on_a;
};
struct alignas(64) TmaGroup {
    CUtensorMap mapA[kMaxGroup];
    CUtensorMap mapB[kMaxGroup];
    TmaProblem p[kMaxGroup];
    int zstart[kMaxGroup + 1];
    int istart[kMaxGroup + 1];
    int count;
};

using namespace tc;

template <int ROWS, bool MN>
__device__ __forceinline__ float raw_at(uint32_t raw, int r, int k) {
    float v;
    asm volatile("ld.shared.f32 %0, [%1];" : "=f"(v) : "r"(raw + 4u * (uint32_t)(MN ? k * ROWS + r : r * 32 + k)));
    return v;
}

template <int ROWS, bool MN, int NT = kThreads>
__device__ __forceinline__ void split_tile(uint32_t raw, uint32_t hi_base, uint32_t lo_base, int klim, int tid) {
    constexpr int kChunks = ROWS * 8;
#pragma unroll
    for (int i = 0; i < (kChunks + NT - 1) / NT; ++i) {
        const int q = tid + i * NT;
        if (q < kChunks) {
            int r, c;
            float4 v;
            if (!MN) {
                r = q >> 3; c = q & 7;
                asm volatile("ld.shared.v4.f32 {%0,%1,%2,%3}, [%4];" : "=f"(v.x), "=f"(v.y), "=f"(v.z), "=f"(v.w)
                             : "r"(raw + 4u * (uint32_t)(r * 32 + 4 * c)));
            } else {
                r = q % ROWS; c = q / ROWS;
                v.x = raw_at<ROWS, true>(raw, r, 4 * c); v.y = raw_at<ROWS, true>(raw, r, 4 * c + 1);
                v.z = raw_at<ROWS, true>(raw, r, 4 * c + 2); v.w = raw_at<ROWS, true>(raw, r, 4 * c + 3);
            }
            if (4 * c >= klim) v.x = 0.f;
            if (4 * c + 1 >= klim) v.y = 0.f;
            if (4 * c + 2 >= klim) v.z = 0.f;
            if (4 * c + 3 >= klim) v.w = 0.f;
            float4 hi, lo;
            hi.x = to_tf32(v.x); hi.y = to_tf32(v.y); hi.z = to_tf32(v.z); hi.w = to_tf32(v.w);
            lo.x = to_tf32(v.x - hi.x); lo.y = to_tf32(v.y - hi.y); lo.z = to_tf32(v.z - hi.z); lo.w = to_tf32(v.w - hi.w);
            const uint32_t off = (uint32_t)(r * 128 + ((c ^ (r & 7)) << 4));
            st_shared_v4(hi_base + off, hi);
            st_shared_v4(lo_base + off, lo);
        }
    }
}

template <int BN>
__device__ __forceinline__ void mma_ss(float (&d)[BN / 2], uint64_t da, uint64_t db) {
    if constexpr (BN == 32) wgmma_ss_n32(d, da, db);
    else wgmma_ss_n64(d, da, db);
}
template <int BN>
__device__ __forceinline__ void mma_rs(float (&d)[BN / 2], const uint32_t (&a)[4], uint64_t db) {
    if constexpr (BN == 32) wgmma_rs_n32(d, a, db);
    else wgmma_rs_n64(d, a, db);
}

template <int BN, bool A_MN, bool B_MN, bool A_REG>
__global__ void __launch_bounds__(kThreads, 1) tma_gemm_kernel(const __grid_constant__ TmaGroup grp) {
    constexpr uint32_t kARaw = 128 * 128, kBRaw = BN * 128;
    constexpr uint32_t kRawStage = kARaw + kBRaw;
    constexpr uint32_t kAHalf = A_REG ? 0 : 128 * 128;
    constexpr uint32_t kSplitStage = 2 * kAHalf + 2 * kBRaw;
    constexpr uint32_t kSplitBase = kNR * kRawStage;
    constexpr int R = BN / 2;
    static_assert(BN == 32 || BN == 64, "BN");

    extern __shared__ __align__(1024) unsigned char smem[];
    __shared__ __align__(8) uint64_t full[kNR];

    int z = blockIdx.z, g = 0;
    if (grp.count > 1 && z >= grp.zstart[1]) g = 1;
    const TmaProblem& P = grp.p[g];
    const CUtensorMap* mapA = &grp.mapA[g];
    const CUtensorMap* mapB = &grp.mapB[g];
    z -= grp.zstart[g];
    const int split = z % P.splitk, batch = z / P.splitk;
    const int m0 = blockIdx.x * 128, n0 = blockIdx.y * BN;
    if (m0 >= P.Ma || n0 >= P.Nb) return;

    const int kbeg = split * P.kchunk;
    const int kend = min(P.K, kbeg + P.kchunk);
    const int nkb = (kend > kbeg) ? (kend - kbeg + kBlockK - 1) / kBlockK : 0;
    const int tid = threadIdx.x, warp = tid >> 5, lane = tid & 31, wg = tid >> 7;
    const uint32_t smem_base = (smem_u32(smem) + 1023u) & ~1023u;

    if (tid == 0) {
        asm volatile("prefetch.tensormap [%0];" ::"l"(mapA) : "memory");
        asm volatile("prefetch.tensormap [%0];" ::"l"(mapB) : "memory");
        for (int s = 0; s < kNR; ++s) mbar_init(&full[s], 1);
        asm volatile("fence.mbarrier_init.release.cluster;" ::: "memory");
    }
    __syncthreads();
    pdl_trigger();
    pdl_wait();

    auto issue = [&](int kb) {
        const int s = kb % kNR;
        const uint32_t raw = smem_base + (uint32_t)s * kRawStage;
        const int k0 = kbeg + kb * kBlockK;
        mbar_expect_tx(&full[s], kRawStage);
        if (A_MN) tma_load_3d(raw, mapA, &full[s], m0, k0, batch);
        else tma_load_3d(raw, mapA, &full[s], k0, m0, batch);
        if (B_MN) tma_load_3d(raw + kARaw, mapB, &full[s], n0, k0, batch);
        else tma_load_3d(raw + kARaw, mapB, &full[s], k0, n0, batch);
    };
    auto split_stage = [&](int kb) {
        mbar_wait(&full[kb % kNR], (uint32_t)((kb / kNR) & 1));
        const uint32_t raw = smem_base + (uint32_t)(kb % kNR) * kRawStage;
        const uint32_t sp = smem_base + kSplitBase + (uint32_t)(kb & 1) * kSplitStage;
        const int klim = kend - (kbeg + kb * kBlockK);
        if (!A_REG) split_tile<128, A_MN>(raw, sp, sp + kAHalf, klim, tid);
        split_tile<BN, B_MN>(raw + kARaw, sp + 2 * kAHalf, sp + 2 * kAHalf + kBRaw, klim, tid);
    };

    float acc0[R], acc1[R], accx[R];
#pragma unroll
    for (int i = 0; i < R; ++i) { acc0[i] = 0.f; acc1[i] = 0.f; accx[i] = 0.f; }
    const int r0 = 64 * wg + 16 * (warp & 3) + (lane >> 2);
    const int q = lane & 3;

    if (nkb > 0) {
        if (tid == 0)
            for (int kb = 0; kb < min(nkb, kNR); ++kb) issue(kb);
        split_stage(0);
    }
    asm volatile("fence.proxy.async.shared::cta;" ::: "memory");
    __syncthreads();
    for (int kb = 0; kb < nkb; ++kb) {
        const uint32_t sp = smem_base + kSplitBase + (uint32_t)(kb & 1) * kSplitStage;
        const uint64_t b_hi = desc_sw128(sp + 2 * kAHalf), b_lo = desc_sw128(sp + 2 * kAHalf + kBRaw);
        if constexpr (A_REG) {
            const uint32_t raw = smem_base + (uint32_t)(kb % kNR) * kRawStage;
            const int klim = kend - (kbeg + kb * kBlockK);
            uint32_t ahi[4][4], alo[4][4];
#pragma unroll
            for (int kk = 0; kk < 4; ++kk) {
#pragma unroll
                for (int f = 0; f < 4; ++f) {
                    const int r = r0 + 8 * (f & 1), k = 8 * kk + q + 4 * (f >> 1);
                    const float x = k < klim ? raw_at<128, A_MN>(raw, r, k) : 0.f;
                    const float h = to_tf32(x);
                    ahi[kk][f] = __float_as_uint(h);
                    alo[kk][f] = __float_as_uint(to_tf32(x - h));
                }
            }
            wgmma_fence();
#pragma unroll
            for (int kk = 0; kk < 4; ++kk) {
                mma_rs<BN>(accx, alo[kk], b_hi + 2 * kk);
                mma_rs<BN>(accx, ahi[kk], b_lo + 2 * kk);
                mma_rs<BN>((kk & 1) ? acc1 : acc0, ahi[kk], b_hi + 2 * kk);
            }
        } else {
            const uint64_t a_hi = desc_sw128(sp + (uint32_t)wg * 8192u), a_lo = desc_sw128(sp + kAHalf + (uint32_t)wg * 8192u);
            wgmma_fence();
#pragma unroll
            for (int kk = 0; kk < 4; ++kk) {
                mma_ss<BN>(accx, a_lo + 2 * kk, b_hi + 2 * kk);
                mma_ss<BN>(accx, a_hi + 2 * kk, b_lo + 2 * kk);
                mma_ss<BN>((kk & 1) ? acc1 : acc0, a_hi + 2 * kk, b_hi + 2 * kk);
            }
        }
        wgmma_commit();
        if (kb + 1 < nkb) split_stage(kb + 1);
        wgmma_wait<0>();
        reg_fence(acc0); reg_fence(acc1); reg_fence(accx);
        asm volatile("fence.proxy.async.shared::cta;" ::: "memory");
        __syncthreads();
        if (tid == 0 && kb + kNR < nkb) issue(kb + kNR);
    }

    const bool add_bias = (P.bias != nullptr) && (split == 0);
    gemm_epilogue(acc0, acc1, accx, P.C + (long long)batch * P.sC + (long long)split * P.strideP, P.c_rs, P.c_cs, P.Ma, P.Nb,
                  m0 + r0, n0 + 2 * q, (add_bias && P.bias_on_a) ? P.bias : nullptr,
                  (add_bias && !P.bias_on_a) ? P.bias : nullptr, P.accumulate != 0);
}

constexpr int kWsThreads = 384;
constexpr int kWsNR = 4, kWsNS = 2;
template <int BN> __host__ __device__ constexpr uint32_t ws_raw() { return 128 * 128 + BN * 128; }
template <int BN> constexpr size_t ws_smem() { return (size_t)kWsNR * ws_raw<BN>() + (size_t)kWsNS * 2 * BN * 128 + 1024; }

struct WsItem { int g, batch, split, m0, n0, kbeg, kend, nkb; };

template <int BN>
__device__ __forceinline__ WsItem ws_item(const TmaGroup& grp, int it) {
    WsItem w;
    w.g = (grp.count > 1 && it >= grp.istart[1]) ? 1 : 0;
    const TmaProblem& P = grp.p[w.g];
    it -= grp.istart[w.g];
    const int mt = (P.Ma + 127) >> 7, nt = (P.Nb + BN - 1) / BN;
    w.m0 = (it % mt) * 128; it /= mt;
    w.n0 = (it % nt) * BN; it /= nt;
    w.split = it % P.splitk; w.batch = it / P.splitk;
    w.kbeg = w.split * P.kchunk;
    w.kend = min(P.K, w.kbeg + P.kchunk);
    w.nkb = (w.kend > w.kbeg) ? (w.kend - w.kbeg + kBlockK - 1) / kBlockK : 0;
    return w;
}

template <bool MN>
__device__ __forceinline__ float raw_a_sw(uint32_t raw, int r, int k) {
    const uint32_t off = MN ? (uint32_t)((r >> 5) * 4096 + k * 128 + ((((r & 31) >> 2) ^ (k & 7)) << 4) + (r & 3) * 4)
                            : (uint32_t)(r * 128 + (((k >> 2) ^ (r & 7)) << 4) + (k & 3) * 4);
    float v;
    asm volatile("ld.shared.f32 %0, [%1];" : "=f"(v) : "r"(raw + off));
    return v;
}
template <int N>
__device__ __forceinline__ void reg_fence_u(uint32_t (&a)[N]) {
#pragma unroll
    for (int i = 0; i < N; ++i) asm volatile("" : "+r"(a[i])::"memory");
}

template <int BN>
__device__ __forceinline__ void mma_rs_ws(float (&d)[BN / 2], const uint32_t (&a)[4], uint64_t db) {
    if constexpr (BN == 96) wgmma_rs_n96(d, a, db);
    else wgmma_rs_n112(d, a, db);
}

template <int BN, bool A_MN, bool B_MN>
__global__ void __launch_bounds__(kWsThreads, 1) tma_gemm_kernel_ws(const __grid_constant__ TmaGroup grp, int items) {
    constexpr uint32_t kRaw = ws_raw<BN>(), kBHalf = BN * 128, kSplit = 2 * kBHalf;
    constexpr int R = BN / 2;
    static_assert(BN == 96 || BN == 112, "BN");
    extern __shared__ __align__(1024) unsigned char smem[];
    __shared__ __align__(8) uint64_t full[kWsNR], empty[kWsNR], sfull[kWsNS], sempty[kWsNS];
    const int tid = threadIdx.x, warp = __shfl_sync(0xffffffffu, tid >> 5, 0), lane = tid & 31;
    const uint32_t smem_base = (smem_u32(smem) + 1023u) & ~1023u;
    const uint32_t split_base = smem_base + kWsNR * kRaw;

    if (tid == 0) {
        for (int g = 0; g < grp.count; ++g) {
            asm volatile("prefetch.tensormap [%0];" ::"l"(&grp.mapA[g]) : "memory");
            asm volatile("prefetch.tensormap [%0];" ::"l"(&grp.mapB[g]) : "memory");
        }
        for (int s = 0; s < kWsNR; ++s) { mbar_init(&full[s], 1); mbar_init(&empty[s], 3 + 8); }
        for (int s = 0; s < kWsNS; ++s) { mbar_init(&sfull[s], 3); mbar_init(&sempty[s], 2); }
        asm volatile("fence.mbarrier_init.release.cluster;" ::: "memory");
    }
    __syncthreads();
    pdl_trigger();
    pdl_wait();

    if (warp < 4) {
        setmaxnreg_dec<64>();
        if (warp == 0) {
            if (lane != 0) return;
            uint32_t kc = 0;
            for (int it = blockIdx.x; it < items; it += gridDim.x) {
                const WsItem w = ws_item<BN>(grp, it);
                const CUtensorMap* mapA = &grp.mapA[w.g];
                const CUtensorMap* mapB = &grp.mapB[w.g];
                for (int kb = 0; kb < w.nkb; ++kb, ++kc) {
                    const int s = kc % kWsNR;
                    mbar_wait(&empty[s], ((kc / kWsNR) & 1) ^ 1);
                    const uint32_t raw = smem_base + (uint32_t)s * kRaw;
                    const int k0 = w.kbeg + kb * kBlockK;
                    mbar_expect_tx(&full[s], kRaw);
                    if (A_MN) {
#pragma unroll
                        for (int j = 0; j < 4; ++j) tma_load_3d(raw + 4096u * j, mapA, &full[s], w.m0 + 32 * j, k0, w.batch);
                    } else {
                        tma_load_3d(raw, mapA, &full[s], k0, w.m0, w.batch);
                    }
                    if (B_MN) tma_load_3d(raw + 128 * 128, mapB, &full[s], w.n0, k0, w.batch);
                    else tma_load_3d(raw + 128 * 128, mapB, &full[s], k0, w.n0, w.batch);
                }
            }
        } else {
            const int stid = tid - 32;
            uint32_t kc = 0;
            for (int it = blockIdx.x; it < items; it += gridDim.x) {
                const WsItem w = ws_item<BN>(grp, it);
                for (int kb = 0; kb < w.nkb; ++kb, ++kc) {
                    const int s = kc % kWsNR, t = kc % kWsNS;
                    mbar_wait(&full[s], (kc / kWsNR) & 1);
                    mbar_wait(&sempty[t], ((kc / kWsNS) & 1) ^ 1);
                    const uint32_t sp = split_base + (uint32_t)t * kSplit;
                    split_tile<BN, B_MN, 96>(smem_base + (uint32_t)s * kRaw + 128 * 128, sp, sp + kBHalf,
                                              w.kend - (w.kbeg + kb * kBlockK), stid);
                    asm volatile("fence.proxy.async.shared::cta;" ::: "memory");
                    __syncwarp();
                    if (lane == 0) { mbar_arrive(&sfull[t]); mbar_arrive(&empty[s]); }
                }
            }
        }
        return;
    }

    setmaxnreg_inc<216>();
    const int ctid = tid - 128, cw = ctid >> 7;
    const int r0 = 64 * cw + 16 * (warp & 3) + (lane >> 2);
    const int q = lane & 3;
    uint32_t kc = 0;
    for (int it = blockIdx.x; it < items; it += gridDim.x) {
        const WsItem w = ws_item<BN>(grp, it);
        const TmaProblem& P = grp.p[w.g];
        float acc0[R], acc1[R], accx[R];
#pragma unroll
        for (int i = 0; i < R; ++i) { acc0[i] = 0.f; acc1[i] = 0.f; accx[i] = 0.f; }
        uint32_t fa[2][2][4] = {};
        for (int kb = 0; kb < w.nkb; ++kb, ++kc) {
            const int s = kc % kWsNR, t = kc % kWsNS;
            mbar_wait(&full[s], (kc / kWsNR) & 1);
            mbar_wait(&sfull[t], (kc / kWsNS) & 1);
            const uint32_t raw = smem_base + (uint32_t)s * kRaw;
            const uint32_t sp = split_base + (uint32_t)t * kSplit;
            const uint64_t b_hi = desc_sw128(sp), b_lo = desc_sw128(sp + kBHalf);
#pragma unroll
            for (int kk = 0; kk < 4; ++kk) {
                uint32_t (&ah)[4] = fa[kk & 1][0];
                uint32_t (&al)[4] = fa[kk & 1][1];
#pragma unroll
                for (int f = 0; f < 4; ++f) {
                    const float x = raw_a_sw<A_MN>(raw, r0 + 8 * (f & 1), 8 * kk + q + 4 * (f >> 1));
                    const float h = to_tf32(x);
                    ah[f] = __float_as_uint(h);
                    al[f] = __float_as_uint(to_tf32(x - h));
                }
                if (kk == 3) {
                    __syncwarp();
                    if (lane == 0) mbar_arrive(&empty[s]);
                }
                wgmma_fence();
                mma_rs_ws<BN>(accx, al, b_hi + 2 * kk);
                mma_rs_ws<BN>(accx, ah, b_lo + 2 * kk);
                mma_rs_ws<BN>((kk & 1) ? acc1 : acc0, ah, b_hi + 2 * kk);
                wgmma_commit();
                wgmma_wait<1>();
                reg_fence_u(fa[(kk + 1) & 1][0]); reg_fence_u(fa[(kk + 1) & 1][1]);
                if (kk == 0 && kb > 0 && (ctid & 127) == 0) mbar_arrive(&sempty[(kc - 1) % kWsNS]);
            }
        }
        wgmma_wait<0>();
        reg_fence(acc0); reg_fence(acc1); reg_fence(accx);
        reg_fence_u(fa[0][0]); reg_fence_u(fa[0][1]); reg_fence_u(fa[1][0]); reg_fence_u(fa[1][1]);
        if (w.nkb > 0 && (ctid & 127) == 0) mbar_arrive(&sempty[(kc - 1) % kWsNS]);
        const bool add_bias = (P.bias != nullptr) && (w.split == 0);
        gemm_epilogue(acc0, acc1, accx, P.C + (long long)w.batch * P.sC + (long long)w.split * P.strideP, P.c_rs, P.c_cs, P.Ma,
                      P.Nb, w.m0 + r0, w.n0 + 2 * q, (add_bias && P.bias_on_a) ? P.bias : nullptr,
                      (add_bias && !P.bias_on_a) ? P.bias : nullptr, P.accumulate != 0);
    }
}

template <int BN, bool A_REG>
constexpr size_t smem_bytes() {
    return (size_t)kNR * (128 * 128 + BN * 128) + 2 * (size_t)(2 * (A_REG ? 0 : 128 * 128) + 2 * BN * 128) + 1024;
}

template <int BN, bool A_REG>
int set_attrs() {
    const int sm = (int)smem_bytes<BN, A_REG>();
    NATS_CUDA_OK(cudaFuncSetAttribute(tma_gemm_kernel<BN, false, false, A_REG>, cudaFuncAttributeMaxDynamicSharedMemorySize, sm));
    NATS_CUDA_OK(cudaFuncSetAttribute(tma_gemm_kernel<BN, false, true, A_REG>, cudaFuncAttributeMaxDynamicSharedMemorySize, sm));
    NATS_CUDA_OK(cudaFuncSetAttribute(tma_gemm_kernel<BN, true, false, A_REG>, cudaFuncAttributeMaxDynamicSharedMemorySize, sm));
    NATS_CUDA_OK(cudaFuncSetAttribute(tma_gemm_kernel<BN, true, true, A_REG>, cudaFuncAttributeMaxDynamicSharedMemorySize, sm));
    return 0;
}

template <int BN, bool A_REG>
int launch_bn(cudaStream_t st, const TmaGroup& grp, bool a_mn, bool b_mn, dim3 grid) {
    const size_t sm = smem_bytes<BN, A_REG>();
    cudaError_t e;
    if (!a_mn && !b_mn) e = launch_pdl(tma_gemm_kernel<BN, false, false, A_REG>, grid, dim3(kThreads), sm, st, grp);
    else if (!a_mn && b_mn) e = launch_pdl(tma_gemm_kernel<BN, false, true, A_REG>, grid, dim3(kThreads), sm, st, grp);
    else if (a_mn && !b_mn) e = launch_pdl(tma_gemm_kernel<BN, true, false, A_REG>, grid, dim3(kThreads), sm, st, grp);
    else e = launch_pdl(tma_gemm_kernel<BN, true, true, A_REG>, grid, dim3(kThreads), sm, st, grp);
    NATS_CUDA_OK(e);
    return 0;
}

int g_num_sms = 0;
int g_ts_mode = 1;

int operand_map(const float* ptr, bool mn, int rows, int K, int ld, int batch, long long bstride, int box_rows, CUtensorMap* out) {
    const long long d0 = mn ? rows : K, d1 = mn ? K : rows;
    return tma_map_tile3d(ptr, d0, d1, batch, ld, batch > 1 ? bstride : d1 * ld, mn ? box_rows : 32, mn ? 32 : box_rows, 1, out);
}

}

bool tma_available() { return g_encode != nullptr; }

namespace {
int encode_tile3d(const float* ptr, long long d0, long long d1, long long d2, long long stride1, long long stride2, int b0, int b1,
                  int b2, bool swizzle128, CUtensorMap* out) {
    NATS_REQUIRE(g_encode != nullptr, "tensor maps not available");
    MapKey key{ptr, d0, d1, stride1, d2, stride2, b0 * 65536 + b1 * 256 + b2, swizzle128 ? 3 : 2};
    auto it = g_maps.find(key);
    if (it != g_maps.end()) { *out = it->second; return 0; }
    if (g_maps.size() > (1u << 16)) g_maps.clear();
    cuuint64_t gdim[3] = {(cuuint64_t)d0, (cuuint64_t)d1, (cuuint64_t)d2};
    cuuint64_t gstr[2] = {(cuuint64_t)stride1 * 4, (cuuint64_t)stride2 * 4};
    cuuint32_t box[3] = {(cuuint32_t)b0, (cuuint32_t)b1, (cuuint32_t)b2};
    cuuint32_t estr[3] = {1, 1, 1};
    CUtensorMap m;
    const CUresult r = g_encode(&m, CU_TENSOR_MAP_DATA_TYPE_FLOAT32, 3, const_cast<float*>(ptr), gdim, gstr, box, estr,
                                CU_TENSOR_MAP_INTERLEAVE_NONE, swizzle128 ? CU_TENSOR_MAP_SWIZZLE_128B : CU_TENSOR_MAP_SWIZZLE_NONE,
                                CU_TENSOR_MAP_L2_PROMOTION_L2_256B, CU_TENSOR_MAP_FLOAT_OOB_FILL_NONE);
    if (r != CUDA_SUCCESS) {
        set_error("cuTensorMapEncodeTiled (tile3d) failed (%d): ptr=%p dims=%lld,%lld,%lld strides=%lld,%lld box=%d,%d,%d", (int)r, ptr, d0,
                  d1, d2, stride1, stride2, b0, b1, b2);
        return 1;
    }
    g_maps.emplace(key, m);
    *out = m;
    return 0;
}

int operand_map_ws_a(const float* ptr, bool mn, int rows, int K, int ld, int batch, long long bstride, CUtensorMap* out) {
    const long long d0 = mn ? rows : K, d1 = mn ? K : rows;
    return encode_tile3d(ptr, d0, d1, batch, ld, batch > 1 ? bstride : d1 * ld, 32, mn ? 32 : 128, 1, true, out);
}

template <int BN>
int set_attrs_ws() {
    const int sm = (int)ws_smem<BN>();
    NATS_CUDA_OK(cudaFuncSetAttribute(tma_gemm_kernel_ws<BN, false, false>, cudaFuncAttributeMaxDynamicSharedMemorySize, sm));
    NATS_CUDA_OK(cudaFuncSetAttribute(tma_gemm_kernel_ws<BN, false, true>, cudaFuncAttributeMaxDynamicSharedMemorySize, sm));
    NATS_CUDA_OK(cudaFuncSetAttribute(tma_gemm_kernel_ws<BN, true, false>, cudaFuncAttributeMaxDynamicSharedMemorySize, sm));
    NATS_CUDA_OK(cudaFuncSetAttribute(tma_gemm_kernel_ws<BN, true, true>, cudaFuncAttributeMaxDynamicSharedMemorySize, sm));
    return 0;
}

template <int BN>
int launch_ws(cudaStream_t st, const TmaGroup& grp, bool a_mn, bool b_mn, int items) {
    const dim3 grid(min(items, g_num_sms)), block(kWsThreads);
    const size_t sm = ws_smem<BN>();
    cudaError_t e;
    if (!a_mn && !b_mn) e = launch_pdl(tma_gemm_kernel_ws<BN, false, false>, grid, block, sm, st, grp, items);
    else if (!a_mn && b_mn) e = launch_pdl(tma_gemm_kernel_ws<BN, false, true>, grid, block, sm, st, grp, items);
    else if (a_mn && !b_mn) e = launch_pdl(tma_gemm_kernel_ws<BN, true, false>, grid, block, sm, st, grp, items);
    else e = launch_pdl(tma_gemm_kernel_ws<BN, true, true>, grid, block, sm, st, grp, items);
    NATS_CUDA_OK(e);
    return 0;
}

}

int tma_map_tile3d(const float* ptr, long long d0, long long d1, long long d2, long long stride1, long long stride2, int b0,
                   int b1, int b2, CUtensorMap* out) {
    return encode_tile3d(ptr, d0, d1, d2, stride1, stride2, b0, b1, b2, false, out);
}
void tma_gemm_set_ts(int on) { g_ts_mode = on; }
int tma_gemm_get_ts() { return g_ts_mode; }

int tma_gemm_setup() {
    void* fn = nullptr;
    cudaDriverEntryPointQueryResult q;
    NATS_CUDA_OK(cudaGetDriverEntryPoint("cuTensorMapEncodeTiled", &fn, cudaEnableDefault, &q));
    if (fn == nullptr || q != cudaDriverEntryPointSuccess) {
        set_error("cuTensorMapEncodeTiled not available from the driver");
        return 1;
    }
    g_encode = reinterpret_cast<EncodeTiledFn>(fn);
    NATS_TRY((set_attrs<32, false>()));
    NATS_TRY((set_attrs<64, false>()));
    NATS_TRY((set_attrs<32, true>()));
    NATS_TRY((set_attrs<64, true>()));
    NATS_TRY(set_attrs_ws<96>());
    NATS_TRY(set_attrs_ws<112>());
    int dev = 0;
    NATS_CUDA_OK(cudaGetDevice(&dev));
    NATS_CUDA_OK(cudaDeviceGetAttribute(&g_num_sms, cudaDevAttrMultiProcessorCount, dev));
    return 0;
}


bool tma_gemm_eligible(const GemmProblem* probs, int count) {
    if (g_encode == nullptr || count > kMaxGroup) return false;
    for (int i = 0; i < count; ++i) {
        const GemmProblem& q = probs[i];
        if ((q.lda & 3) || (q.ldb & 3)) return false;
        if ((reinterpret_cast<uintptr_t>(q.A) & 15) || (reinterpret_cast<uintptr_t>(q.B) & 15)) return false;
        if (q.batch > 1 && ((q.strideA & 3) || (q.strideB & 3))) return false;
        if (q.M < 1 || q.N < 1 || q.K < 1) return false;
    }
    return true;
}

int tma_gemm_launch(cudaStream_t st, const GemmProblem* probs, int count, bool transA, bool transB) {
    NATS_REQUIRE(count >= 1 && count <= kMaxGroup, "tma gemm group size");
    TmaGroup grp;
    memset(&grp, 0, sizeof(grp));
    grp.count = count;
    int maxM = 0, maxN = 0;
    for (int i = 0; i < count; ++i) { maxM = max(maxM, probs[i].M); maxN = max(maxN, probs[i].N); }
    const bool swapped = maxM < 128 && maxN > maxM;
    const int nb_dim = swapped ? maxM : maxN;
    const bool skinny = nb_dim <= 64;
    const int BN = nb_dim <= 32 ? 32 : nb_dim <= 64 ? 64 : nb_dim <= 112 ? 112 : 96;
    const bool opa_mn = transA, opb_mn = !transB;
    const bool a_mn = swapped ? opb_mn : opa_mn;
    const bool b_mn = swapped ? opa_mn : opb_mn;
    int z = 0, ga = 0, gb = 0, items = 0;
    double flops = 0.0, bytes = 0.0;
    for (int i = 0; i < count; ++i) {
        const GemmProblem& q = probs[i];
        NATS_REQUIRE(q.splitk >= 1 && q.batch >= 1 && (q.splitk == 1 || !q.accumulate), "tma gemm split/batch");
        TmaProblem& t = grp.p[i];
        const float* pa = swapped ? q.B : q.A;
        const float* pb = swapped ? q.A : q.B;
        const int rows_a = swapped ? q.N : q.M, rows_b = swapped ? q.M : q.N;
        const int ld_a = swapped ? q.ldb : q.lda, ld_b = swapped ? q.lda : q.ldb;
        const long long s_a = swapped ? q.strideB : q.strideA, s_b = swapped ? q.strideA : q.strideB;
        if (skinny) NATS_TRY(operand_map(pa, a_mn, rows_a, q.K, ld_a, q.batch, s_a, 128, &grp.mapA[i]));
        else NATS_TRY(operand_map_ws_a(pa, a_mn, rows_a, q.K, ld_a, q.batch, s_a, &grp.mapA[i]));
        NATS_TRY(operand_map(pb, b_mn, rows_b, q.K, ld_b, q.batch, s_b, BN, &grp.mapB[i]));
        t.Ma = rows_a; t.Nb = rows_b;
        if (!swapped) { t.c_rs = q.ldc; t.c_cs = 1; t.bias_on_a = 0; }
        else { t.c_rs = 1; t.c_cs = q.ldc; t.bias_on_a = 1; }
        t.C = q.C; t.bias = q.bias; t.K = q.K; t.batch = q.batch; t.sC = q.strideC;
        t.splitk = q.splitk;
        t.kchunk = ((q.kchunk + 31) / 32) * 32;
        if (q.splitk > 1) t.kchunk = ((cdiv(q.K, q.splitk) + 31) / 32) * 32;
        if (t.kchunk <= 0) t.kchunk = 32;
        t.strideP = q.strideP; t.accumulate = q.accumulate;
        grp.zstart[i] = z;
        grp.istart[i] = items;
        z += q.batch * q.splitk;
        items += q.batch * q.splitk * cdiv(t.Ma, 128) * cdiv(t.Nb, BN);
        ga = max(ga, cdiv(t.Ma, 128));
        gb = max(gb, cdiv(t.Nb, BN));
        flops += 2.0 * q.M * q.N * q.K * q.batch;
        bytes += 4.0 * q.batch * ((double)q.M * q.K + (double)q.K * q.N + (double)q.M * q.N * q.splitk);
    }
    grp.zstart[count] = z;
    grp.istart[count] = items;
    for (int i = count; i < kMaxGroup; ++i) { grp.zstart[i + 1] = z; grp.istart[i + 1] = items; }
    if (items == 0) return 0;
    ProfScope ps(st, skinny ? K_TC_GEMM_SKINNY : K_TC_GEMM, flops, bytes);
    if (BN == 112) return launch_ws<112>(st, grp, a_mn, b_mn, items);
    if (BN == 96) return launch_ws<96>(st, grp, a_mn, b_mn, items);
    dim3 grid(ga, gb, z);
    const bool areg = g_ts_mode != 0;
    if (BN == 32) return areg ? launch_bn<32, true>(st, grp, a_mn, b_mn, grid) : launch_bn<32, false>(st, grp, a_mn, b_mn, grid);
    return areg ? launch_bn<64, true>(st, grp, a_mn, b_mn, grid) : launch_bn<64, false>(st, grp, a_mn, b_mn, grid);
}

}
```

Measured before the change: 36480.

## Replace skinny TMA GEMM with TS kernel that prefetches constant weights before PDL wait

Replaces the skinny-path TMA GEMM with a new kernel. B is split into TF32 hi/lo tiles directly from global memory into a resident shared buffer. A streams through a TMA ring that uses empty/full mbarriers. GEMM calls whose weight operand is constant are flagged b_const, so when operands are swapped the weight loads are issued before the programmatic-dependent-launch wait, overlapping them with the previous kernel's tail. The change also pipelines per-kk wgmma commits and drops the SS/register toggle. It adds complexity around shared-memory budgeting and barrier handling, and exposes a debug entry point.

Measured after the change: 37920 (median of 6 runs). +4.0%, better.

```diff
diff --git a/include/nats_b200.h b/include/nats_b200.h
--- a/include/nats_b200.h
+++ b/include/nats_b200.h
@@ -156,6 +156,9 @@
 int nats_debug_gemm(nats_ctx_t* ctx, void* stream, int path, int transA, int transB, int M, int N, int K,
                     const float* A, int lda, const float* B, int ldb, float* C, int ldc, const float* bias,
                     int accumulate, int splitk, int batch, int64_t strideA, int64_t strideB, int64_t strideC);
+int nats_debug_gemm_const_b(nats_ctx_t* ctx, void* stream, int transA, int transB, int M, int N, int K, const float* A,
+                            int lda, const float* B, int ldb, float* C, int ldc, int splitk, int b_const,
+                            const float* A_src);
 
 int nats_profile_enable(nats_ctx_t* ctx, int on);
 int nats_profile_num_classes(void);
diff --git a/nats_b200/_lib.py b/nats_b200/_lib.py
--- a/nats_b200/_lib.py
+++ b/nats_b200/_lib.py
@@ -84,6 +84,8 @@
     'nats_beam_step_many': (c_int, [c_void_p, _P, POINTER(Dims), POINTER(BeamStepMany), c_int]),
     'nats_debug_gemm': (c_int, [c_void_p, _P, c_int, c_int, c_int, c_int, c_int, c_int, _P, c_int, _P, c_int, _P, c_int,
                                 _P, c_int, c_int, c_int, c_int64, c_int64, c_int64]),
+    'nats_debug_gemm_const_b': (c_int, [c_void_p, _P, c_int, c_int, c_int, c_int, c_int, _P, c_int, _P, c_int, _P, c_int,
+                                        c_int, c_int, _P]),
     'nats_profile_enable': (c_int, [c_void_p, c_int]),
     'nats_profile_num_classes': (c_int, []),
     'nats_profile_class_name': (c_char_p, [c_int]),
diff --git a/nats_b200/csrc/api.cu b/nats_b200/csrc/api.cu
--- a/nats_b200/csrc/api.cu
+++ b/nats_b200/csrc/api.cu
@@ -53,6 +53,13 @@
 static int g_pdl = 1;
 int pdl_enabled() { return g_pdl; }
 void pdl_set(int on) { g_pdl = on; }
+
+__global__ void debug_copy_kernel(const float* src, float* dst, long long n) {
+    pdl_trigger();
+    pdl_wait();
+    for (long long i = blockIdx.x * (long long)blockDim.x + threadIdx.x; i < n; i += (long long)gridDim.x * blockDim.x)
+        dst[i] = src[i];
+}
 }
 
 using namespace nats;
@@ -97,7 +104,6 @@
     if (r == 0) r = enc_tc_setup(c);
     enc_tc_enable(getenv("NATS_ENC_TC") ? atoi(getenv("NATS_ENC_TC")) : 1);
     attention_set_cc_keep(getenv("NATS_CC_KEEP") ? atoi(getenv("NATS_CC_KEEP")) : 0);
-    tma_gemm_set_ts(getenv("NATS_TS") ? atoi(getenv("NATS_TS")) : 1);
     if (getenv("NATS_TRACE_GATES")) gates_trace(atoi(getenv("NATS_TRACE_GATES")));
     pdl_set(getenv("NATS_PDL") ? atoi(getenv("NATS_PDL")) : 1);
     gemm_set_tensor_cores(getenv("NATS_TC") ? atoi(getenv("NATS_TC")) : 2);
@@ -187,17 +193,29 @@
     if (path == 1) return tc_gemm_launch(st, &p, 1, transA != 0, transB != 0);
     if (path == 2 || path == 3) {
         NATS_REQUIRE(tma_gemm_eligible(&p, 1), "operands not TMA-compatible (alignment)");
-        const int keep_ts = tma_gemm_get_ts();
-        tma_gemm_set_ts(path == 3 ? 1 : 0);
-        const int r = tma_gemm_launch(st, &p, 1, transA != 0, transB != 0);
-        tma_gemm_set_ts(keep_ts);
-        return r;
+        return tma_gemm_launch(st, &p, 1, transA != 0, transB != 0);
     }
     const int keep = gemm_get_tensor_cores();
     gemm_set_tensor_cores(0);
     const int r = gemm_launch(st, &p, 1, transA != 0, transB != 0, GEMM_CFG_AUTO);
     gemm_set_tensor_cores(keep);
     return r;
+}
+
+int nats_debug_gemm_const_b(nats_ctx_t* ctx, void* stream, int transA, int transB, int M, int N, int K, const float* A,
+                            int lda, const float* B, int ldb, float* C, int ldc, int splitk, int b_const,
+                            const float* A_src) {
+    NATS_REQUIRE(ctx && A && B && C, "null argument");
+    GemmProblem p = gemm_problem(A, lda, B, ldb, C, ldc, M, N, K);
+    if (splitk > 1) gemm_set_split(p, splitk, (long long)M * ldc);
+    p.b_const = b_const;
+    NATS_REQUIRE(tma_gemm_eligible(&p, 1), "operands not TMA-compatible (alignment)");
+    cudaStream_t st = reinterpret_cast<cudaStream_t>(stream);
+    if (A_src) {
+        const long long n = (long long)(transA ? K : M) * lda;
+        NATS_CUDA_OK(launch_pdl(debug_copy_kernel, dim3(132), dim3(256), 0, st, A_src, const_cast<float*>(A), n));
+    }
+    return tma_gemm_launch(st, &p, 1, transA != 0, transB != 0);
 }
 
 int nats_profile_enable(nats_ctx_t* ctx, int on) {
@@ -394,6 +412,7 @@
     {
         GemmProblem p = gemm_problem(w.emb_y, W, params + o.dec.Wcat, D3, w.xproj_y, D3, n, D3, W);
         p.bias = params + o.dec.bcat;
+        p.b_const = 1;
         NATS_TRY(gemm_auto(ctx, st, p, false, false, w.gemm_scratch, w.gemm_scratch_floats));
     }
     const float* pctx = pctx_in;
@@ -409,6 +428,7 @@
             pts = (long long)n * A; pbs = A;
         }
         p.bias = params + o.b_att;
+        p.b_const = 1;
         NATS_TRY(gemm_auto(ctx, st, p, false, false, w.gemm_scratch, w.gemm_scratch_floats));
         pctx = w.pctx;
     }
@@ -438,18 +458,19 @@
         NATS_TRY(narrow_proj(st, np));
     } else {
         p = gemm_problem(state_out, D, params + o.lstm_W, W, w.L, W, n, W, D);
-        p.bias = params + o.lstm_b;
+        p.bias = params + o.lstm_b; p.b_const = 1;
         NATS_TRY(gemm_auto(ctx, st, p, false, false, w.gemm_scratch, w.gemm_scratch_floats));
         p = gemm_problem(w.emb_y, W, params + o.prev_W, W, w.L, W, n, W, W);
-        p.bias = params + o.prev_b; p.accumulate = 1;
+        p.bias = params + o.prev_b; p.accumulate = 1; p.b_const = 1;
         NATS_TRY(gemm_auto(ctx, st, p, false, false, w.gemm_scratch, w.gemm_scratch_floats));
         p = gemm_problem(ctxs, C, params + o.ctxr_W, W, w.L, W, n, W, C);
-        p.bias = params + o.ctxr_b; p.accumulate = 1;
+        p.bias = params + o.ctxr_b; p.accumulate = 1; p.b_const = 1;
         NATS_TRY(gemm_auto(ctx, st, p, false, false, w.gemm_scratch, w.gemm_scratch_floats));
         NATS_TRY(tanh_inplace(st, w.L, (long long)n * W));
     }
     p = gemm_problem(w.L, W, params + o.logit_W, V, w.logits, V, n, V, W);
     p.bias = params + o.logit_b;
+    p.b_const = 1;
     NATS_TRY(gemm_auto(ctx, st, p, false, false, w.gemm_scratch, w.gemm_scratch_floats));
     NATS_TRY(softmax_sample_rows(st, w.logits, n, V, probs, sample, rng_seed, rng_step));
     return 0;
diff --git a/nats_b200/csrc/gemm.cuh b/nats_b200/csrc/gemm.cuh
--- a/nats_b200/csrc/gemm.cuh
+++ b/nats_b200/csrc/gemm.cuh
@@ -17,6 +17,7 @@
     int kchunk;
     long long strideP;
     int accumulate;
+    int b_const;
 };
 
 constexpr int kGemmMaxGroup = 4;
diff --git a/nats_b200/csrc/model_bwd.cu b/nats_b200/csrc/model_bwd.cu
--- a/nats_b200/csrc/model_bwd.cu
+++ b/nats_b200/csrc/model_bwd.cu
@@ -71,6 +71,7 @@
             gemm_set_split(q[0], SA, spD);
             q[1] = gemm_problem(w.dG1x + r3, D3, params + o.W1cat, D3, w.part_a, C, B, C, D3);
             gemm_set_split(q[1], SB, spC);
+            q[0].b_const = q[1].b_const = 1;
             NATS_TRY(gemm_launch(st, q, 2, false, true, cfg));
         }
         {
@@ -98,6 +99,7 @@
         }
         {
             GemmProblem q = gemm_problem(w.dps + rA, A, params + o.W_att, A, w.part_d, D, B, D, A);
+            q.b_const = 1;
             NATS_TRY(gemm_launch(st, &q, 1, false, true, cfg));
         }
         {
@@ -115,6 +117,7 @@
         {
             GemmProblem q = gemm_problem(w.dG2 + r3, D3, params + o.dec.Ucat, D3, w.part_c, D, B, D, D3);
             gemm_set_split(q, S4, spD);
+            q.b_const = 1;
             NATS_TRY(gemm_launch(st, &q, 1, false, true, cfg));
         }
     }
@@ -216,6 +219,7 @@
                 q[dir] = gemm_problem(w.dGe[dir] + (long long)pos * B * D3, D3, params + o.enc[dir].Ucat, D3,
                                       w.part_a + (long long)dir * B * D, D, B, D, D3);
                 gemm_set_split(q[dir], S, strideP);
+                q[dir].b_const = 1;
             }
             NATS_TRY(gemm_launch(st, q, 2, false, true, cfg));
         }
diff --git a/nats_b200/csrc/model_fwd.cu b/nats_b200/csrc/model_fwd.cu
--- a/nats_b200/csrc/model_fwd.cu
+++ b/nats_b200/csrc/model_fwd.cu
@@ -42,6 +42,7 @@
                                     e.part_a + (long long)n * D3, D3, n, D3, D);
                 gemm_set_split(q[0], S, strideP);
                 gemm_set_split(q[1], S, strideP);
+                q[0].b_const = q[1].b_const = 1;
                 NATS_TRY(gemm_launch(st, q, 2, false, false, cfg));
             }
             GateFwd g[2];
@@ -88,6 +89,7 @@
     {
         GemmProblem q = gemm_problem(s.h_prev, D, params + o.dec.Ucat, D3, s.part_b, D3, n, D3, D);
         gemm_set_split(q, S1, sp3);
+        q.b_const = 1;
         NATS_TRY(gemm_launch(st, &q, 1, false, false, cfg));
         GateFwd g;
         memset(&g, 0, sizeof(g));
@@ -105,6 +107,7 @@
         gemm_set_split(q[0], S1, sp3);
         q[1] = gemm_problem(s.h1, D, params + o.W_att, A, s.part_d, A, n, A, D);
         gemm_set_split(q[1], S1, (long long)n * A);
+        q[0].b_const = q[1].b_const = 1;
         NATS_TRY(gemm_launch(st, q, 2, false, false, cfg));
     }
     {
@@ -128,6 +131,7 @@
     {
         GemmProblem q = gemm_problem(s.ctx_out, C, params + o.W1cat, D3, s.part_a, D3, n, D3, C);
         gemm_set_split(q, S2, sp3);
+        q.b_const = 1;
         NATS_TRY(gemm_launch(st, &q, 1, false, false, cfg));
         GateFwd g;
         memset(&g, 0, sizeof(g));
diff --git a/nats_b200/csrc/ops.cuh b/nats_b200/csrc/ops.cuh
--- a/nats_b200/csrc/ops.cuh
+++ b/nats_b200/csrc/ops.cuh
@@ -68,8 +68,6 @@
 long long enc_tc_counter_ints();
 int enc_tc_fwd(const nats_ctx* ctx, cudaStream_t st, const EncTcFwdArgs& a);
 int enc_tc_bwd(const nats_ctx* ctx, cudaStream_t st, const EncTcBwdArgs& a);
-void tma_gemm_set_ts(int on);
-int tma_gemm_get_ts();
 void gates_trace(int on);
 void attention_set_cc_keep(int mode);
 
diff --git a/nats_b200/csrc/tma_gemm.cu b/nats_b200/csrc/tma_gemm.cu
--- a/nats_b200/csrc/tma_gemm.cu
+++ b/nats_b200/csrc/tma_gemm.cu
@@ -35,12 +35,13 @@
 
 constexpr int kThreads = 256;
 constexpr int kBlockK = 32;
-constexpr int kNR = 3;
 constexpr int kMaxGroup = 2;
 
 struct TmaProblem {
     float* C;
     const float* bias;
+    const float* B;
+    long long ldb, sB;
     int Ma, Nb, K;
     long long c_rs, c_cs;
     int batch;
@@ -49,6 +50,7 @@
     long long strideP;
     int accumulate;
     int bias_on_a;
+    int a_pre;
 };
 struct alignas(64) TmaGroup {
     CUtensorMap mapA[kMaxGroup];
@@ -57,6 +59,7 @@
     int zstart[kMaxGroup + 1];
     int istart[kMaxGroup + 1];
     int count;
+    int ts_na, ts_rb;
 };
 
 using namespace tc;
@@ -98,138 +101,6 @@
             st_shared_v4(lo_base + off, lo);
         }
     }
-}
-
-template <int BN>
-__device__ __forceinline__ void mma_ss(float (&d)[BN / 2], uint64_t da, uint64_t db) {
-    if constexpr (BN == 32) wgmma_ss_n32(d, da, db);
-    else wgmma_ss_n64(d, da, db);
-}
-template <int BN>
-__device__ __forceinline__ void mma_rs(float (&d)[BN / 2], const uint32_t (&a)[4], uint64_t db) {
-    if constexpr (BN == 32) wgmma_rs_n32(d, a, db);
-    else wgmma_rs_n64(d, a, db);
-}
-
-template <int BN, bool A_MN, bool B_MN, bool A_REG>
-__global__ void __launch_bounds__(kThreads, 1) tma_gemm_kernel(const __grid_constant__ TmaGroup grp) {
-    constexpr uint32_t kARaw = 128 * 128, kBRaw = BN * 128;
-    constexpr uint32_t kRawStage = kARaw + kBRaw;
-    constexpr uint32_t kAHalf = A_REG ? 0 : 128 * 128;
-    constexpr uint32_t kSplitStage = 2 * kAHalf + 2 * kBRaw;
-    constexpr uint32_t kSplitBase = kNR * kRawStage;
-    constexpr int R = BN / 2;
-    static_assert(BN == 32 || BN == 64, "BN");
-
-    extern __shared__ __align__(1024) unsigned char smem[];
-    __shared__ __align__(8) uint64_t full[kNR];
-
-    int z = blockIdx.z, g = 0;
-    if (grp.count > 1 && z >= grp.zstart[1]) g = 1;
-    const TmaProblem& P = grp.p[g];
-    const CUtensorMap* mapA = &grp.mapA[g];
-    const CUtensorMap* mapB = &grp.mapB[g];
-    z -= grp.zstart[g];
-    const int split = z % P.splitk, batch = z / P.splitk;
-    const int m0 = blockIdx.x * 128, n0 = blockIdx.y * BN;
-    if (m0 >= P.Ma || n0 >= P.Nb) return;
-
-    const int kbeg = split * P.kchunk;
-    const int kend = min(P.K, kbeg + P.kchunk);
-    const int nkb = (kend > kbeg) ? (kend - kbeg + kBlockK - 1) / kBlockK : 0;
-    const int tid = threadIdx.x, warp = tid >> 5, lane = tid & 31, wg = tid >> 7;
-    const uint32_t smem_base = (smem_u32(smem) + 1023u) & ~1023u;
-
-    if (tid == 0) {
-        asm volatile("prefetch.tensormap [%0];" ::"l"(mapA) : "memory");
-        asm volatile("prefetch.tensormap [%0];" ::"l"(mapB) : "memory");
-        for (int s = 0; s < kNR; ++s) mbar_init(&full[s], 1);
-        asm volatile("fence.mbarrier_init.release.cluster;" ::: "memory");
-    }
-    __syncthreads();
-    pdl_trigger();
-    pdl_wait();
-
-    auto issue = [&](int kb) {
-        const int s = kb % kNR;
-        const uint32_t raw = smem_base + (uint32_t)s * kRawStage;
-        const int k0 = kbeg + kb * kBlockK;
-        mbar_expect_tx(&full[s], kRawStage);
-        if (A_MN) tma_load_3d(raw, mapA, &full[s], m0, k0, batch);
-        else tma_load_3d(raw, mapA, &full[s], k0, m0, batch);
-        if (B_MN) tma_load_3d(raw + kARaw, mapB, &full[s], n0, k0, batch);
-        else tma_load_3d(raw + kARaw, mapB, &full[s], k0, n0, batch);
-    };
-    auto split_stage = [&](int kb) {
-        mbar_wait(&full[kb % kNR], (uint32_t)((kb / kNR) & 1));
-        const uint32_t raw = smem_base + (uint32_t)(kb % kNR) * kRawStage;
-        const uint32_t sp = smem_base + kSplitBase + (uint32_t)(kb & 1) * kSplitStage;
-        const int klim = kend - (kbeg + kb * kBlockK);
-        if (!A_REG) split_tile<128, A_MN>(raw, sp, sp + kAHalf, klim, tid);
-        split_tile<BN, B_MN>(raw + kARaw, sp + 2 * kAHalf, sp + 2 * kAHalf + kBRaw, klim, tid);
-    };
-
-    float acc0[R], acc1[R], accx[R];
-#pragma unroll
-    for (int i = 0; i < R; ++i) { acc0[i] = 0.f; acc1[i] = 0.f; accx[i] = 0.f; }
-    const int r0 = 64 * wg + 16 * (warp & 3) + (lane >> 2);
-    const int q = lane & 3;
-
-    if (nkb > 0) {
-        if (tid == 0)
-            for (int kb = 0; kb < min(nkb, kNR); ++kb) issue(kb);
-        split_stage(0);
-    }
-    asm volatile("fence.proxy.async.shared::cta;" ::: "memory");
-    __syncthreads();
-    for (int kb = 0; kb < nkb; ++kb) {
-        const uint32_t sp = smem_base + kSplitBase + (uint32_t)(kb & 1) * kSplitStage;
-        const uint64_t b_hi = desc_sw128(sp + 2 * kAHalf), b_lo = desc_sw128(sp + 2 * kAHalf + kBRaw);
-        if constexpr (A_REG) {
-            const uint32_t raw = smem_base + (uint32_t)(kb % kNR) * kRawStage;
-            const int klim = kend - (kbeg + kb * kBlockK);
-            uint32_t ahi[4][4], alo[4][4];
-#pragma unroll
-            for (int kk = 0; kk < 4; ++kk) {
-#pragma unroll
-                for (int f = 0; f < 4; ++f) {
-                    const int r = r0 + 8 * (f & 1), k = 8 * kk + q + 4 * (f >> 1);
-                    const float x = k < klim ? raw_at<128, A_MN>(raw, r, k) : 0.f;
-                    const float h = to_tf32(x);
-                    ahi[kk][f] = __float_as_uint(h);
-                    alo[kk][f] = __float_as_uint(to_tf32(x - h));
-                }
-            }
-            wgmma_fence();
-#pragma unroll
-            for (int kk = 0; kk < 4; ++kk) {
-                mma_rs<BN>(accx, alo[kk], b_hi + 2 * kk);
-                mma_rs<BN>(accx, ahi[kk], b_lo + 2 * kk);
-                mma_rs<BN>((kk & 1) ? acc1 : acc0, ahi[kk], b_hi + 2 * kk);
-            }
-        } else {
-            const uint64_t a_hi = desc_sw128(sp + (uint32_t)wg * 8192u), a_lo = desc_sw128(sp + kAHalf + (uint32_t)wg * 8192u);
-            wgmma_fence();
-#pragma unroll
-            for (int kk = 0; kk < 4; ++kk) {
-                mma_ss<BN>(accx, a_lo + 2 * kk, b_hi + 2 * kk);
-                mma_ss<BN>(accx, a_hi + 2 * kk, b_lo + 2 * kk);
-                mma_ss<BN>((kk & 1) ? acc1 : acc0, a_hi + 2 * kk, b_hi + 2 * kk);
-            }
-        }
-        wgmma_commit();
-        if (kb + 1 < nkb) split_stage(kb + 1);
-        wgmma_wait<0>();
-        reg_fence(acc0); reg_fence(acc1); reg_fence(accx);
-        asm volatile("fence.proxy.async.shared::cta;" ::: "memory");
-        __syncthreads();
-        if (tid == 0 && kb + kNR < nkb) issue(kb + kNR);
-    }
-
-    const bool add_bias = (P.bias != nullptr) && (split == 0);
-    gemm_epilogue(acc0, acc1, accx, P.C + (long long)batch * P.sC + (long long)split * P.strideP, P.c_rs, P.c_cs, P.Ma, P.Nb,
-                  m0 + r0, n0 + 2 * q, (add_bias && P.bias_on_a) ? P.bias : nullptr,
-                  (add_bias && !P.bias_on_a) ? P.bias : nullptr, P.accumulate != 0);
 }
 
 constexpr int kWsThreads = 384;
@@ -400,35 +271,200 @@
     }
 }
 
-template <int BN, bool A_REG>
-constexpr size_t smem_bytes() {
-    return (size_t)kNR * (128 * 128 + BN * 128) + 2 * (size_t)(2 * (A_REG ? 0 : 128 * 128) + 2 * BN * 128) + 1024;
-}
-
-template <int BN, bool A_REG>
-int set_attrs() {
-    const int sm = (int)smem_bytes<BN, A_REG>();
-    NATS_CUDA_OK(cudaFuncSetAttribute(tma_gemm_kernel<BN, false, false, A_REG>, cudaFuncAttributeMaxDynamicSharedMemorySize, sm));
-    NATS_CUDA_OK(cudaFuncSetAttribute(tma_gemm_kernel<BN, false, true, A_REG>, cudaFuncAttributeMaxDynamicSharedMemorySize, sm));
-    NATS_CUDA_OK(cudaFuncSetAttribute(tma_gemm_kernel<BN, true, false, A_REG>, cudaFuncAttributeMaxDynamicSharedMemorySize, sm));
-    NATS_CUDA_OK(cudaFuncSetAttribute(tma_gemm_kernel<BN, true, true, A_REG>, cudaFuncAttributeMaxDynamicSharedMemorySize, sm));
+constexpr uint32_t kTsASlot = 128 * 128;
+constexpr int kTsMaxSlots = 14;
+constexpr size_t kTsSmemMax = 227 * 1024 - 1024;
+
+template <int BN, bool MN>
+__device__ __forceinline__ void split_b_global(const float* b, long long ld, int rows, int n0, int k0, int kend, int nkb,
+                                               uint32_t base, int tid) {
+    constexpr int kPerKb = BN * 8;
+    constexpr int kU = 4;
+    const int total = nkb * kPerKb;
+    for (int q0 = 0; q0 < total; q0 += kU * kThreads) {
+        float4 v[kU];
+#pragma unroll
+        for (int i = 0; i < kU; ++i) {
+            const int q = q0 + i * kThreads + tid, w = q % kPerKb;
+            const int r = MN ? w % BN : w >> 3, c = MN ? w / BN : w & 7;
+            const int n = n0 + r, k = k0 + (q / kPerKb) * kBlockK + 4 * c;
+            float t[4] = {0.f, 0.f, 0.f, 0.f};
+            if (q < total && n < rows) {
+                if (!MN && k + 3 < kend) {
+                    const float4 x = *reinterpret_cast<const float4*>(b + (long long)n * ld + k);
+                    t[0] = x.x; t[1] = x.y; t[2] = x.z; t[3] = x.w;
+                } else {
+#pragma unroll
+                    for (int j = 0; j < 4; ++j)
+                        if (k + j < kend) t[j] = MN ? b[(long long)(k + j) * ld + n] : b[(long long)n * ld + k + j];
+                }
+            }
+            v[i] = make_float4(t[0], t[1], t[2], t[3]);
+        }
+#pragma unroll
+        for (int i = 0; i < kU; ++i) {
+            const int q = q0 + i * kThreads + tid, w = q % kPerKb;
+            if (q < total) {
+                const int r = MN ? w % BN : w >> 3, c = MN ? w / BN : w & 7;
+                float4 hi, lo;
+                hi.x = to_tf32(v[i].x); hi.y = to_tf32(v[i].y); hi.z = to_tf32(v[i].z); hi.w = to_tf32(v[i].w);
+                lo.x = to_tf32(v[i].x - hi.x); lo.y = to_tf32(v[i].y - hi.y);
+                lo.z = to_tf32(v[i].z - hi.z); lo.w = to_tf32(v[i].w - hi.w);
+                const uint32_t off = base + (uint32_t)(q / kPerKb) * (2 * BN * 128) + (uint32_t)(r * 128 + ((c ^ (r & 7)) << 4));
+                st_shared_v4(off, hi);
+                st_shared_v4(off + BN * 128, lo);
+            }
+        }
+    }
+}
+
+template <int BN>
+__device__ __forceinline__ void mma_rs(float (&d)[BN / 2], const uint32_t (&a)[4], uint64_t db) {
+    if constexpr (BN == 32) wgmma_rs_n32(d, a, db);
+    else wgmma_rs_n64(d, a, db);
+}
+
+template <int BN, bool A_MN, bool B_MN>
+__global__ void __launch_bounds__(kThreads, 1) tma_gemm_ts_kernel(const __grid_constant__ TmaGroup grp) {
+    constexpr uint32_t kBHalf = BN * 128, kBTile = 2 * kBHalf;
+    constexpr int R = BN / 2;
+    static_assert(BN == 32 || BN == 64, "BN");
+    extern __shared__ __align__(1024) unsigned char smem[];
+    __shared__ __align__(8) uint64_t full[kTsMaxSlots], empty[kTsMaxSlots];
+
+    int z = blockIdx.z, g = 0;
+    if (grp.count > 1 && z >= grp.zstart[1]) g = 1;
+    const TmaProblem& P = grp.p[g];
+    const CUtensorMap* mapA = &grp.mapA[g];
+    z -= grp.zstart[g];
+    const int split = z % P.splitk, batch = z / P.splitk;
+    const int m0 = blockIdx.x * 128, n0 = blockIdx.y * BN;
+    if (m0 >= P.Ma || n0 >= P.Nb) return;
+
+    const int kbeg = split * P.kchunk;
+    const int kend = min(P.K, kbeg + P.kchunk);
+    const int nkb = (kend > kbeg) ? (kend - kbeg + kBlockK - 1) / kBlockK : 0;
+    const int na = grp.ts_na, rb = grp.ts_rb;
+    const int tid = threadIdx.x, warp = tid >> 5, lane = tid & 31, wg = tid >> 7;
+    const uint32_t b_base = (smem_u32(smem) + 1023u) & ~1023u;
+    const uint32_t a_base = b_base + (uint32_t)rb * kBTile;
+
+    if (tid == 0) {
+        asm volatile("prefetch.tensormap [%0];" ::"l"(mapA) : "memory");
+        for (int s = 0; s < na; ++s) { mbar_init(&full[s], 1); mbar_init(&empty[s], kThreads / 32); }
+        asm volatile("fence.mbarrier_init.release.cluster;" ::: "memory");
+    }
+    __syncthreads();
+    pdl_trigger();
+
+    auto issue = [&](int kb) {
+        const int s = kb % na;
+        const uint32_t raw = a_base + (uint32_t)s * kTsASlot;
+        const int k0 = kbeg + kb * kBlockK;
+        mbar_expect_tx(&full[s], kTsASlot);
+        if (A_MN) {
+#pragma unroll
+            for (int j = 0; j < 4; ++j) tma_load_3d(raw + 4096u * j, mapA, &full[s], m0 + 32 * j, k0, batch);
+        } else {
+            tma_load_3d(raw, mapA, &full[s], k0, m0, batch);
+        }
+    };
+    const int npre = min(nkb, na);
+    if (tid == 0 && P.a_pre)
+        for (int kb = 0; kb < npre; ++kb) issue(kb);
+    pdl_wait();
+    if (tid == 0 && !P.a_pre)
+        for (int kb = 0; kb < npre; ++kb) issue(kb);
+
+    float acc0[R], acc1[R], accx[R];
+#pragma unroll
+    for (int i = 0; i < R; ++i) { acc0[i] = 0.f; acc1[i] = 0.f; accx[i] = 0.f; }
+    const int r0 = 64 * wg + 16 * (warp & 3) + (lane >> 2);
+    const int q = lane & 3;
+    const float* bsrc = P.B + (long long)batch * P.sB;
+    uint32_t fa[2][2][4] = {};
+    for (int kr = 0; kr < nkb; kr += rb) {
+        const int nr = min(rb, nkb - kr);
+        if (kr > 0) {
+            wgmma_wait<0>();
+            reg_fence(acc0); reg_fence(acc1); reg_fence(accx);
+            __syncthreads();
+        }
+        split_b_global<BN, B_MN>(bsrc, P.ldb, P.Nb, n0, kbeg + kr * kBlockK, kend, nr, b_base, tid);
+        asm volatile("fence.proxy.async.shared::cta;" ::: "memory");
+        __syncthreads();
+        for (int kb = kr; kb < kr + nr; ++kb) {
+            const int s = kb % na;
+            mbar_wait(&full[s], (uint32_t)((kb / na) & 1));
+            const uint32_t raw = a_base + (uint32_t)s * kTsASlot;
+            const uint32_t bt = b_base + (uint32_t)(kb - kr) * kBTile;
+            const uint64_t b_hi = desc_sw128(bt), b_lo = desc_sw128(bt + kBHalf);
+#pragma unroll
+            for (int kk = 0; kk < 4; ++kk) {
+                uint32_t (&ah)[4] = fa[kk & 1][0];
+                uint32_t (&al)[4] = fa[kk & 1][1];
+#pragma unroll
+                for (int f = 0; f < 4; ++f) {
+                    const float x = raw_a_sw<A_MN>(raw, r0 + 8 * (f & 1), 8 * kk + q + 4 * (f >> 1));
+                    const float h = to_tf32(x);
+                    ah[f] = __float_as_uint(h);
+                    al[f] = __float_as_uint(to_tf32(x - h));
+                }
+                if (kk == 3) {
+                    __syncwarp();
+                    if (lane == 0) mbar_arrive(&empty[s]);
+                }
+                wgmma_fence();
+                mma_rs<BN>(accx, al, b_hi + 2 * kk);
+                mma_rs<BN>(accx, ah, b_lo + 2 * kk);
+                mma_rs<BN>((kk & 1) ? acc1 : acc0, ah, b_hi + 2 * kk);
+                wgmma_commit();
+                wgmma_wait<1>();
+                reg_fence_u(fa[(kk + 1) & 1][0]); reg_fence_u(fa[(kk + 1) & 1][1]);
+            }
+            if (tid == 0 && kb + na < nkb) {
+                mbar_wait(&empty[s], (uint32_t)((kb / na) & 1));
+                issue(kb + na);
+            }
+        }
+    }
+    wgmma_wait<0>();
+    reg_fence(acc0); reg_fence(acc1); reg_fence(accx);
+    reg_fence_u(fa[0][0]); reg_fence_u(fa[0][1]); reg_fence_u(fa[1][0]); reg_fence_u(fa[1][1]);
+
+    const bool add_bias = (P.bias != nullptr) && (split == 0);
+    gemm_epilogue(acc0, acc1, accx, P.C + (long long)batch * P.sC + (long long)split * P.strideP, P.c_rs, P.c_cs, P.Ma, P.Nb,
+                  m0 + r0, n0 + 2 * q, (add_bias && P.bias_on_a) ? P.bias : nullptr,
+                  (add_bias && !P.bias_on_a) ? P.bias : nullptr, P.accumulate != 0);
+}
+
+template <int BN>
+int set_attrs_ts() {
+    const int sm = (int)kTsSmemMax;
+    NATS_CUDA_OK(cudaFuncSetAttribute(tma_gemm_ts_kernel<BN, false, false>, cudaFuncAttributeMaxDynamicSharedMemorySize, sm));
+    NATS_CUDA_OK(cudaFuncSetAttribute(tma_gemm_ts_kernel<BN, false, true>, cudaFuncAttributeMaxDynamicSharedMemorySize, sm));
+    NATS_CUDA_OK(cudaFuncSetAttribute(tma_gemm_ts_kernel<BN, true, false>, cudaFuncAttributeMaxDynamicSharedMemorySize, sm));
+    NATS_CUDA_OK(cudaFuncSetAttribute(tma_gemm_ts_kernel<BN, true, true>, cudaFuncAttributeMaxDynamicSharedMemorySize, sm));
     return 0;
 }
 
-template <int BN, bool A_REG>
-int launch_bn(cudaStream_t st, const TmaGroup& grp, bool a_mn, bool b_mn, dim3 grid) {
-    const size_t sm = smem_bytes<BN, A_REG>();
+template <int BN>
+int launch_ts(cudaStream_t st, TmaGroup& grp, bool a_mn, bool b_mn, dim3 grid, int nkb) {
+    const size_t budget = kTsSmemMax - 1024, bt = 2 * BN * 128;
+    const int rb = (int)std::min<size_t>((size_t)nkb, (budget - 4 * kTsASlot) / bt);
+    const int na = (int)std::min<size_t>((size_t)std::min(nkb, kTsMaxSlots), (budget - rb * bt) / kTsASlot);
+    grp.ts_rb = rb; grp.ts_na = na;
+    const size_t sm = rb * bt + (size_t)na * kTsASlot + 1024;
     cudaError_t e;
-    if (!a_mn && !b_mn) e = launch_pdl(tma_gemm_kernel<BN, false, false, A_REG>, grid, dim3(kThreads), sm, st, grp);
-    else if (!a_mn && b_mn) e = launch_pdl(tma_gemm_kernel<BN, false, true, A_REG>, grid, dim3(kThreads), sm, st, grp);
-    else if (a_mn && !b_mn) e = launch_pdl(tma_gemm_kernel<BN, true, false, A_REG>, grid, dim3(kThreads), sm, st, grp);
-    else e = launch_pdl(tma_gemm_kernel<BN, true, true, A_REG>, grid, dim3(kThreads), sm, st, grp);
+    if (!a_mn && !b_mn) e = launch_pdl(tma_gemm_ts_kernel<BN, false, false>, grid, dim3(kThreads), sm, st, grp);
+    else if (!a_mn && b_mn) e = launch_pdl(tma_gemm_ts_kernel<BN, false, true>, grid, dim3(kThreads), sm, st, grp);
+    else if (a_mn && !b_mn) e = launch_pdl(tma_gemm_ts_kernel<BN, true, false>, grid, dim3(kThreads), sm, st, grp);
+    else e = launch_pdl(tma_gemm_ts_kernel<BN, true, true>, grid, dim3(kThreads), sm, st, grp);
     NATS_CUDA_OK(e);
     return 0;
 }
 
 int g_num_sms = 0;
-int g_ts_mode = 1;
 
 int operand_map(const float* ptr, bool mn, int rows, int K, int ld, int batch, long long bstride, int box_rows, CUtensorMap* out) {
     const long long d0 = mn ? rows : K, d1 = mn ? K : rows;
@@ -499,8 +535,6 @@
                    int b1, int b2, CUtensorMap* out) {
     return encode_tile3d(ptr, d0, d1, d2, stride1, stride2, b0, b1, b2, false, out);
 }
-void tma_gemm_set_ts(int on) { g_ts_mode = on; }
-int tma_gemm_get_ts() { return g_ts_mode; }
 
 int tma_gemm_setup() {
     void* fn = nullptr;
@@ -511,10 +545,8 @@
         return 1;
     }
     g_encode = reinterpret_cast<EncodeTiledFn>(fn);
-    NATS_TRY((set_attrs<32, false>()));
-    NATS_TRY((set_attrs<64, false>()));
-    NATS_TRY((set_attrs<32, true>()));
-    NATS_TRY((set_attrs<64, true>()));
+    NATS_TRY(set_attrs_ts<32>());
+    NATS_TRY(set_attrs_ts<64>());
     NATS_TRY(set_attrs_ws<96>());
     NATS_TRY(set_attrs_ws<112>());
     int dev = 0;
@@ -550,7 +582,7 @@
     const bool opa_mn = transA, opb_mn = !transB;
     const bool a_mn = swapped ? opb_mn : opa_mn;
     const bool b_mn = swapped ? opa_mn : opb_mn;
-    int z = 0, ga = 0, gb = 0, items = 0;
+    int z = 0, ga = 0, gb = 0, items = 0, nkb = 1;
     double flops = 0.0, bytes = 0.0;
     for (int i = 0; i < count; ++i) {
         const GemmProblem& q = probs[i];
@@ -561,9 +593,10 @@
         const int rows_a = swapped ? q.N : q.M, rows_b = swapped ? q.M : q.N;
         const int ld_a = swapped ? q.ldb : q.lda, ld_b = swapped ? q.lda : q.ldb;
         const long long s_a = swapped ? q.strideB : q.strideA, s_b = swapped ? q.strideA : q.strideB;
-        if (skinny) NATS_TRY(operand_map(pa, a_mn, rows_a, q.K, ld_a, q.batch, s_a, 128, &grp.mapA[i]));
-        else NATS_TRY(operand_map_ws_a(pa, a_mn, rows_a, q.K, ld_a, q.batch, s_a, &grp.mapA[i]));
-        NATS_TRY(operand_map(pb, b_mn, rows_b, q.K, ld_b, q.batch, s_b, BN, &grp.mapB[i]));
+        NATS_TRY(operand_map_ws_a(pa, a_mn, rows_a, q.K, ld_a, q.batch, s_a, &grp.mapA[i]));
+        if (!skinny) NATS_TRY(operand_map(pb, b_mn, rows_b, q.K, ld_b, q.batch, s_b, BN, &grp.mapB[i]));
+        t.B = pb; t.ldb = ld_b; t.sB = s_b;
+        t.a_pre = swapped && q.b_const;
         t.Ma = rows_a; t.Nb = rows_b;
         if (!swapped) { t.c_rs = q.ldc; t.c_cs = 1; t.bias_on_a = 0; }
         else { t.c_rs = 1; t.c_cs = q.ldc; t.bias_on_a = 1; }
@@ -572,6 +605,7 @@
         t.kchunk = ((q.kchunk + 31) / 32) * 32;
         if (q.splitk > 1) t.kchunk = ((cdiv(q.K, q.splitk) + 31) / 32) * 32;
         if (t.kchunk <= 0) t.kchunk = 32;
+        nkb = max(nkb, cdiv(min(t.kchunk, t.K), kBlockK));
         t.strideP = q.strideP; t.accumulate = q.accumulate;
         grp.zstart[i] = z;
         grp.istart[i] = items;
@@ -590,9 +624,8 @@
     if (BN == 112) return launch_ws<112>(st, grp, a_mn, b_mn, items);
     if (BN == 96) return launch_ws<96>(st, grp, a_mn, b_mn, items);
     dim3 grid(ga, gb, z);
-    const bool areg = g_ts_mode != 0;
-    if (BN == 32) return areg ? launch_bn<32, true>(st, grp, a_mn, b_mn, grid) : launch_bn<32, false>(st, grp, a_mn, b_mn, grid);
-    return areg ? launch_bn<64, true>(st, grp, a_mn, b_mn, grid) : launch_bn<64, false>(st, grp, a_mn, b_mn, grid);
-}
-
-}
+    if (BN == 32) return launch_ts<32>(st, grp, a_mn, b_mn, grid, nkb);
+    return launch_ts<64>(st, grp, a_mn, b_mn, grid, nkb);
+}
+
+}
```
